# tjhladish/AbcSmc

Hardware: AMD Instinct MI355X
Metric: particles/sec per SMC generation (PLS+weight+resample), 1/2/4/8 GPU (higher is better)
Workload: dtype f64 (inputs, model, distances, proposals, results; pair sums of the weight stage: fp64 operands as three f16 limbs on the matrix pipe + f32 v_exp_f32, weights <= 5e-7 rel of the fp64 oracle, largest seen 3.1e-7); 1 GPU; configs[2]: synthetic 1M particles x 16 params x 32 metrics, PLS 8 components, full generation; particles_per_gpu=1000000, particles_total=1000000, metrics=32, params=16, pls_components=8, pred_prior_size=100000, prev_pred_prior_size=100000, next_set_size=1000000, noise=MULTIVARIATE, ncomp_chosen=8, pls_component_rule=wilcoxon, parallelism=row-sharded x1, launcher=single GPU

## Files before the change

abcsmc_amd/csrc/abc_internal.h:

```cpp
#pragma once
#include <hip/hip_runtime.h>
#include <stddef.h>
#include <stdint.h>
#include <stdio.h>
#include <stdlib.h>
#include <string.h>

#include "../../include/abcsmc_hip.h"

#define ABC_WAVE 64

inline const char* abc_diag_env(const char* name) {
    static const bool on = [] { const char* d = getenv("ABC_DIAG"); return d && d[0] == '1'; }();
    return on ? getenv(name) : nullptr;
}

struct abc_wx_words {
    int left;
    int vmax_lo, vmax_hi;
    int ncomp;
    int changed;
    int decided;
    int n_rest;
    int n_level;
// ... 205 lines not shown
}

int launch_stats_shift(abc_ctx*, const double* X, const double* Y, size_t n, size_t ldx, size_t ldy,
                       size_t M, size_t P, double* stats);
bool abc_gram_takes_i8(const abc_ctx*, const double* X, const double* Y, size_t n, size_t ldx, size_t ldy, size_t M, size_t P,
                       uint64_t n_train_global, size_t n_set);
int launch_stats_accumulate(abc_ctx*, const double* X, const double* Y, size_t n, size_t ldx,
                            size_t ldy, size_t M, size_t P, uint64_t row0, uint64_t n_train_global,
                            double* stats, size_t n_set = 0);
int launch_pls_model(abc_ctx*, const double* stats, const double* obs, size_t M, size_t P, size_t A,
                     int rule, double* model, hipEvent_t done = nullptr);
int launch_simple_model(abc_ctx*, const double* stats, const double* obs, size_t M, size_t P,
                        double* model);
int launch_project_distance(abc_ctx*, const double* X, size_t n, size_t ldx, size_t M, size_t P,
                            size_t A, const double* model, int simple, double* dist);
size_t launch_project_scores(abc_ctx*, const double* X, size_t n, size_t ldx, size_t M, size_t P, size_t A, const double* model, double* S);
int launch_project_distance_scores(abc_ctx*, const double* X, size_t n, size_t ldx, size_t M, size_t P, size_t A, const double* model,
                                   double* dist, double* S, size_t sld, size_t row_test, hipEvent_t done);
int launch_distance_from_scores(abc_ctx*, const double* S, size_t n, size_t sld, size_t M, size_t P, size_t A, const double* model, double* dist);
size_t abc_targets_need(size_t N, size_t A, size_t B, size_t K, bool any_excl);
struct abc_tg_scores { const double* S; size_t sld; const double* O; int KCO; };
int launch_rank_targets(abc_ctx*, const double* X, size_t ldx, const double* Y, size_t ldy, size_t N, size_t M, size_t P,
                        const double* model, size_t A, const double* targets, size_t ldt, size_t B, const uint64_t* exclude,
                        bool any_excl, size_t K, uint64_t* idx, double* dist, double* post_mean, abc_tg_scores* keep = nullptr,
                        const double* om = nullptr);
int launch_row_weights_check(abc_ctx*, const double* w_dev, size_t N, double* out4_dev);
size_t abc_adjust_need(size_t N, size_t A, size_t P, size_t B, size_t K, bool hcorr = false, size_t ridge = 0);
int launch_rank_targets_adjust(abc_ctx*, const double* X, size_t ldx, const double* Y, size_t ldy, size_t N, size_t M, size_t P,
                               const double* model, size_t A, const double* targets, size_t ldt, size_t B, const uint64_t* exclude,
                               bool any_excl, size_t K, int kernel, uint64_t* idx, double* dist, const abc_adjust_out* out,
                               struct abc_adj_keep* keep = nullptr, const struct AbcTf* tf = nullptr,
                               const struct AbcHc* hc = nullptr, const struct AbcRg* rg = nullptr, const double* om = nullptr);
size_t abc_path_need(size_t N, size_t A, size_t P, size_t B, size_t K, size_t T, bool hcorr = false, size_t ridge = 0);
int launch_rank_targets_path(abc_ctx*, const double* X, size_t ldx, const double* Y, size_t ldy, size_t N, size_t M, size_t P,
                             const double* model, size_t A, const double* targets, size_t ldt, size_t B, const uint64_t* exclude,
                             bool any_excl, int kernel, uint64_t* idx, double* dist, const abc_path* path,
                             struct abc_adj_keep* keep = nullptr, const double* Yt = nullptr, const struct AbcTf* tf = nullptr,
                             const struct AbcHc* hc = nullptr, const struct AbcRg* rg = nullptr, const double* om = nullptr);
int launch_param_transf(abc_ctx*, const struct AbcTf* tf, const double* V, size_t ldv, size_t n, size_t P, int inverse, double* out,
                        size_t ldo, unsigned long long* outside);
struct SmValues {
    int method;
    const uint64_t* idx;
    const double* Y;
    size_t ldy;
    const struct abc_adj_keep* adj;
    int A;
    int kernel;
    const double* V;
    size_t ldv;
    const double* w;
    const double* om;
};
size_t abc_summary_need(size_t B, size_t K, size_t P);
int launch_summary(abc_ctx*, const SmValues& sv, size_t B, size_t K, size_t P, const abc_summary* sum);
size_t abc_path_summary_need(size_t B, const size_t* Ks, size_t T, size_t P, int method);
int launch_path_summary(abc_ctx*, const SmValues& sv, size_t B, const size_t* Ks, size_t T, size_t P, const abc_summary* sum);
int abc_summary_check_weights(abc_ctx*, const double* w, size_t K, const char* fn);
size_t abc_density_need(size_t B, size_t K, size_t P, size_t G);
int launch_density(abc_ctx*, const SmValues& sv, size_t B, size_t K, size_t P, const abc_density* dn, const char* fn);
struct DnSeg;
size_t abc_density_segs_need(size_t B, size_t K, size_t P);
int launch_density_segs(abc_ctx*, const SmValues& sv, size_t B, size_t K, size_t P, const abc_density* dn, const DnSeg** segs,
                        const char* fn);
size_t abc_joint_pairs(const abc_joint* jt, size_t P);
size_t abc_joint_need(size_t B, size_t K, size_t P, size_t G, size_t npairs);
int launch_joint(abc_ctx*, const SmValues& sv, size_t B, size_t K, size_t P, const abc_joint* jt, const char* fn);
size_t abc_draws_need(size_t B, size_t K, size_t P, int smooth);
int launch_draws(abc_ctx*, const SmValues& sv, size_t B, size_t K, size_t P, const abc_draws* dr, const char* fn);
int launch_select_smallest(abc_ctx*, const double* dist, size_t n, size_t K, uint64_t idx_base,
                           uint64_t* idx, double* dist_out, bool defer_check = false);
int abc_select_check(abc_ctx* ctx, int* failed);
int abc_select_check_queue(abc_ctx* ctx, int* slot);
int abc_select_check_done(abc_ctx* ctx, const int* slot);
inline size_t abc_kde_slices(size_t kn, size_t Kp, int PP) {
    if (kn == 0 || Kp == 0) return 1;
    size_t rows_per_slice = 24576 / (size_t)PP;
    if (rows_per_slice < 256) rows_per_slice = 256;
    size_t s = (Kp + rows_per_slice - 1) / rows_per_slice;
    const size_t rb = (kn + 255) / 256;
    if (s * rb < 4096) s = (4096 + rb - 1) / rb;
    size_t cap = ((size_t)64 << 20) / (8 * kn);
    if (cap < 8) cap = 8;
    if (s > cap) s = cap;
    if (s > Kp / 64) s = Kp / 64;
    if (s < 1) s = 1;
    if (s > 1024) s = 1024;
    return s;
}
int launch_merge_runs(abc_ctx* ctx, const double* key, const uint64_t* idx, int W, size_t len, double* okey, uint64_t* oidx,
                      uint64_t* osrc = nullptr);
int launch_sort_pairs(abc_ctx*, double* key, uint64_t* idx, size_t n);
int launch_select_begin(abc_ctx*, uint64_t K, long long* state, int* hist);
int launch_select_hist(abc_ctx*, const double* dist, size_t n, const long long* state, int pass, int* hist);
int launch_select_pick(abc_ctx*, long long* state, int pass, int* hist, uint64_t K);
int launch_select_count(abc_ctx*, const double* dist, size_t n, const long long* state, long long* counts);
int launch_select_compact(abc_ctx*, const double* dist, size_t n, const long long* state, uint64_t n_less,
                          uint64_t ties_take, uint64_t idx_base, uint64_t* idx_out, double* dist_out);
int abc_sort_u64_bytes(abc_ctx*, unsigned long long* key0, unsigned long long* val0, unsigned long long* key1,
                       unsigned long long* val1, size_t n, int byte_lo, int byte_hi);
struct abc_wx_shard {
    size_t nv_total;
    const double* nv_ranks;
    size_t nv_stride;
};
bool abc_wx_cascade_applies(size_t nv_total, size_t P, size_t A);
int launch_wilcoxon(abc_ctx*, const double* X, const double* Y, size_t n, size_t ldx, size_t ldy, size_t M, size_t P,
                    size_t A, size_t row_test, double* model, const abc_wx_shard* sh = nullptr, double* dec = nullptr,
                    int* changed_host = nullptr, int stop_at_max = 0);
int launch_wilcoxon_commit(abc_ctx*, double* model, size_t M, size_t P, size_t A, const double* dec, int with_hdr);
struct abc_wx_run;
struct abc_wx_scores_hook { int (*fn)(void* arg, double** S, size_t* sld); void* arg; };
int launch_wilcoxon_begin(abc_ctx*, const double* X, const double* Y, size_t n, size_t ldx, size_t ldy, size_t M, size_t P, size_t A,
                          size_t row_test, double* model, double* dec, int stop_at_max, abc_wx_run** out,
                          const abc_wx_scores_hook* scores = nullptr, int hold_level0 = 0, const abc_wx_shard* sh = nullptr);
int launch_wilcoxon_level0(abc_ctx*, abc_wx_run* run);
int launch_wilcoxon_finish(abc_ctx*, abc_wx_run* run, int* changed_host);
void launch_wilcoxon_abandon(abc_ctx*, abc_wx_run* run, hipStream_t its_stream);
int abc_comm_all_reduce(abc_ctx* ctx, void* buf, size_t count, int dtype);
int abc_comm_all_gather(abc_ctx* ctx, const void* send, void* recv, size_t bytes);
int abc_xbuf_reserve(abc_ctx* ctx, size_t bytes);
int abc_giveups_ensure(abc_ctx* ctx);
int launch_gather_rows(abc_ctx*, const double* Y, size_t n_local, size_t ldy, size_t P,
                       const uint64_t* idx, size_t K, uint64_t idx_base, double* theta, size_t ldt,
                       const int* sel_fail = nullptr, int* sel_fail_pin = nullptr, hipEvent_t done = nullptr);
#define ABC_INTERNAL_RETRY (-2147483647)
int launch_doubled_variance(abc_ctx*, const double* theta, size_t K, size_t P, double* dv);
int launch_theta_stats(abc_ctx*, const double* theta, size_t K, size_t P, double** stats_out);
struct abc_theta_fused {
    double* dv; double* L; int* spd; double* rows ; double* Lpad ;
    const double* model_hdr; double* hdr_pin; int* spd_pin;
};
int launch_post_tail(abc_ctx*, const double* theta, size_t K, size_t P, const double* stats, const abc_theta_fused* f);
int launch_dv_from_stats(abc_ctx*, const double* stats, size_t P, double* dv);
int launch_mvn_from_stats(abc_ctx*, const double* stats, size_t P, double* L, int* status_dev);
struct abc_wprev {
    void* wc ; double* b; double* hb; unsigned short* bt; unsigned* far_list;
    unsigned* tmin;
    size_t Kp, P, kn_max; int split, ready;
};
int launch_weights_prev(abc_ctx*, size_t P, size_t kn_max, const double* theta_prev, size_t Kp, const double* w_prev,
                        const double* dv_prev, abc_wprev* out, hipStream_t st);
int launch_weights_raw(abc_ctx*, const abc_prior* priors, const double* theta, size_t K, size_t P,
                       size_t k0, size_t kn, const double* theta_prev, size_t Kp,
                       const double* w_prev, const double* dv_prev, double* w_raw, const abc_wprev* prev = nullptr,
                       const double** sumsq_out = nullptr);
int abc_weights_prev_early(abc_ctx* ctx, size_t P, size_t kn_max, const double* theta_prev, size_t Kp, const double* w_prev,
                           const double* dv_prev, abc_wprev* out);
int launch_fill(abc_ctx*, double* w, size_t K, double v, hipStream_t st = nullptr);
int launch_normalize_l2(abc_ctx*, double* w, size_t K, double* host_mirror = nullptr, const double* sumsq_parts = nullptr);
static inline size_t abc_alias_pin_bytes(size_t K) { return K * (sizeof(double) * 3 + sizeof(uint32_t) * 3) + 2 * sizeof(uint32_t) + 16; }
int launch_mvn_setup(abc_ctx*, const double* theta, size_t K, size_t P, double* L, int* status_host,
                     int* status_dev);
int launch_resample(abc_ctx*, const abc_rng* rng, const double* w, size_t K, uint64_t i0, size_t n,
                    uint64_t* parent, int (*while_host_builds)(void*) = nullptr, void* hook_arg = nullptr,
                    bool uniform_weights = false, const uint32_t* raw_ready = nullptr, bool weights_on_host = false,
                    const volatile int* abort_flag = nullptr, bool parents_ready = false, int* alias_check_deferred = nullptr);
int abc_rng_streams_early(abc_ctx* ctx, const abc_rng* rng, uint64_t i0, size_t n, uint64_t* seeds, uint64_t seed_stream_offset,
                          uint32_t** raw, uint64_t* parent_uniform = nullptr, size_t K_uniform = 0);
int abc_rng_seeds_early(abc_ctx* ctx, const abc_rng* rng, uint64_t i0, size_t n, uint64_t* seeds, uint64_t seed_stream_offset);
int abc_side_fork(abc_ctx* ctx);
int abc_uniform_alias(abc_ctx* ctx, size_t K);
struct abc_perturb_prep { double* rows; int seeds_done; double* Lpad; };
int launch_perturb_prepare(abc_ctx*, const abc_rng* rng, const double* theta, size_t K, size_t P, uint64_t i0, size_t n,
                           uint64_t* seeds, uint64_t seed_stream_offset, abc_perturb_prep* prep, int multivariate = 0,
                           const double* L_or_dv = nullptr);
static inline int abc_perturb_pp(size_t P) {
    int PP = 2;
    while (PP < (int)P) PP *= 2;
    return (P > 64) ? (int)((P + 63) / 64 * 64) : PP;
}
int launch_perturb(abc_ctx*, const abc_rng* rng, const double* theta, size_t K, size_t P,
                   const abc_prior* priors, const uint64_t* parent, uint64_t i0, size_t n,
                   int multivariate, const double* L_or_dv, double* out, uint64_t* seeds,
                   uint64_t seed_stream_offset, const abc_perturb_prep* prep = nullptr);

struct abc_side_moments { abc_theta_fused out; double* stats; double* L; };
int abc_moments_on_side(abc_ctx* ctx, const double* theta, size_t K, size_t P, bool multivariate, double* L_io, double* dv,
                        int* spd_dev, const double* model_hdr, bool theta_ev_bound, const char* who, abc_side_moments* m);
int abc_normalize_for_resample(abc_ctx* ctx, double* w, size_t K, size_t Nn, const double* sumsq, bool* w_on_host);
struct abc_prep_arg {
    abc_ctx* ctx; const abc_rng* rng; const double* theta; const double* theta_stats; size_t K, P, Nn;
    uint64_t i0, seed_off; uint64_t* seeds; abc_perturb_prep* prep; double* L; int* spd_dev; double* dv; bool moments;
    const double* model_hdr; double* hdr_pin; int* spd_pin;
};
int abc_prep_hook(void* prep_arg);
int abc_alias_repair(abc_ctx* ctx, const abc_rng* rng_entry, const double* w, size_t K, uint64_t i0, size_t Nn, uint64_t seed_off,
                     uint64_t* parent, const double* theta, size_t P, const abc_prior* priors, int multivariate, const double* L_or_dv,
                     double* next, abc_perturb_prep* prep, bool giveups_to_snapshot);

int launch_perturb_reference(abc_ctx*, abc_rng* rng_after_draws, const double* theta, size_t K, size_t P, const abc_prior* priors,
                             const uint64_t* parent, size_t n, int multivariate, const double* L_or_dv, double* out,
                             uint64_t* seeds);

void abc_alias_preproc(size_t K, const double* w, double* F, uint32_t* A, double* E, uint32_t* smalls, uint32_t* bigs, bool knuth = true);

int launch_alias_build_dev(abc_ctx*, const double* w, size_t K, double* F, uint32_t* A, int* fail_dev, int* fail_pin,
                           const int** verdict_src = nullptr);
size_t abc_alias_dev_need(size_t K);
constexpr size_t ABC_ALIAS_DEV_MAX_K = (size_t)2 << 20;
constexpr size_t ABC_ALIAS_DEV_MIN_K = 20000;
constexpr size_t ABC_ALIAS_DEV_SMALL_K = 300000;

size_t abc_ws_need(size_t N, size_t M, size_t P, size_t A, size_t K, size_t Kp, size_t Nnext);
size_t abc_wx_need(size_t n_validation, size_t P, size_t A);
int abc_timing_flush(abc_ctx* ctx);
void abc_comm_release(abc_ctx* ctx);

void taus2_set(abc_rng* r, unsigned long seed);
uint32_t taus2_get(abc_rng* r);
void taus2_jump(abc_rng* r, uint64_t n);
```

abcsmc_amd/csrc/alias_dev.hip:

```cpp
#include <stdlib.h>

#include "abc_internal.h"

namespace {

typedef __int128 i128;
typedef unsigned __int128 u128;
typedef unsigned long long u64;

#ifndef ABC_AL_I
#define ABC_AL_I 4
#endif
#define ABC_AL_CAT2(a, b) a##b
#define ABC_AL_CAT(a, b) ABC_AL_CAT2(a, b)
#define ABC_AL_FN(name) ABC_AL_CAT(name##_i, ABC_AL_I)
constexpr int AL_T = 256;
constexpr int AL_I = ABC_AL_I;
constexpr int AL_B = AL_T * AL_I;
constexpr int AL_MAXBLK = 8192;
constexpr int AL_SUM_BITS = 44;

struct RMap { i128 t0, t1, b; int k; int pad_[3]; };

__device__ __forceinline__ i128 shl(i128 v, int s) { return (i128)((u128)v << s); }
__device__ __forceinline__ int bitlen(i128 v) {
    const u64 hi = (u64)((u128)v >> 64), lo = (u64)v;
    return hi ? 128 - __clzll((long long)hi) : (lo ? 64 - __clzll((long long)lo) : 0);
}
__device__ __forceinline__ int level_of(i128 v) { const int b = bitlen(v); return b > 53 ? b - 53 : 0; }

__device__ __forceinline__ RMap rne_map(int k, i128 c, bool sticky) {
    RMap m;
    m.k = k; m.b = 0; m.pad_[0] = m.pad_[1] = m.pad_[2] = 0;
    if (k == 0) { m.t0 = -c - 1; m.t1 = -c; return m; }
    const i128 P = shl(1, k + 1), h = shl(1, k - 1);
    const i128 t_even = -c - shl(1, k) + h;
    const i128 t_odd = -c + h + (sticky ? 0 : 1);
    m.t0 = t_odd - P; m.t1 = t_even;
    return m;
}
__device__ __forceinline__ RMap rmap_identity() { RMap m; m.k = 0; m.t0 = -1; m.t1 = 0; m.b = 0; m.pad_[0] = m.pad_[1] = m.pad_[2] = 0; return m; }
__device__ __forceinline__ i128 rapply(const RMap& m, i128 y) {
    return shl(((y - m.t0) >> (m.k + 1)) + ((y - m.t1) >> (m.k + 1)), m.k) + m.b;
}
__device__ __forceinline__ i128 inv_min(const RMap& m, i128 v) {
    const i128 a = -((-(v - m.b)) >> m.k);
    if (a & 1) return m.t0 + shl((a + 1) >> 1, m.k + 1);
    return m.t1 + shl(a >> 1, m.k + 1);
}
__device__ __forceinline__ RMap compose(const RMap& m1, const RMap& m2) {
    RMap r;
    if (m2.k < m1.k) { r = m1; r.b = rapply(m2, m1.b); return r; }
    r.k = m2.k; r.t0 = inv_min(m1, m2.t0); r.t1 = inv_min(m1, m2.t1); r.b = m2.b;
    r.pad_[0] = r.pad_[1] = r.pad_[2] = 0;
    return r;
}

__device__ __forceinline__ i128 to_grid(double x, int e0, bool* inexact) {
    const u64 bits = (u64)__double_as_longlong(x);
    const int be = (int)((bits >> 52) & 0x7ff);
    u64 mant = bits & 0xfffffffffffffull;
    int e;
    if (be == 0) { if (mant == 0) return 0; e = -1074; } else { mant |= 1ull << 52; e = be - 1075; }
    const int sh = e - e0;
    if (sh >= 0) return (sh < 70) ? shl((i128)mant, sh) : (i128)0;
    if (sh <= -64) { *inexact = true; return 0; }
    if (mant & ((1ull << -sh) - 1)) *inexact = true;
    return (i128)(mant >> -sh);
}
__device__ __forceinline__ double from_grid(i128 v, int e0, bool* ok) {
    if (v < 0) { *ok = false; return 0.0; }
    if (v == 0) return 0.0;
    const int bl = bitlen(v), sh = bl > 53 ? bl - 53 : 0;
    const u64 top = (u64)(v >> sh);
    if (shl((i128)top, sh) != v) { *ok = false; return 0.0; }
    return ldexp((double)top, sh + e0);
}

__device__ __forceinline__ i128 shfl_up_i128(i128 v, int d) {
    const u64 lo = (u64)__shfl_up((long long)(u64)v, d, 64), hi = (u64)__shfl_up((long long)(u64)((u128)v >> 64), d, 64);
    return (i128)(((u128)hi << 64) | lo);
}
__device__ __forceinline__ RMap shfl_up_map(const RMap& m, int d) {
    RMap r;
    r.t0 = shfl_up_i128(m.t0, d); r.t1 = shfl_up_i128(m.t1, d); r.b = shfl_up_i128(m.b, d); r.k = __shfl_up(m.k, d, 64);
    r.pad_[0] = r.pad_[1] = r.pad_[2] = 0;
    return r;
}
__device__ __forceinline__ RMap block_scan_maps(RMap mine, RMap (*buf)[AL_T], RMap* excl) {
    const int t = threadIdx.x, lane = t & 63, wave = t >> 6;
    RMap inc = mine;
#pragma unroll
    for (int d = 1; d < 64; d <<= 1) {
        const RMap up = shfl_up_map(inc, d);
        if (lane >= d) inc = compose(up, inc);
    }
    RMap exw = shfl_up_map(inc, 1);
    if (lane == 0) exw = rmap_identity();
    if (lane == 63) buf[0][wave] = inc;
    __syncthreads();
    RMap before = rmap_identity();
    for (int w = 0; w < wave; w++) before = compose(before, buf[0][w]);
    __syncthreads();
    *excl = compose(before, exw);
    return compose(before, inc);
}
__device__ __forceinline__ RMap prefix_of_blocks(const RMap* __restrict__ agg, int nb, RMap (*buf)[AL_T]) {
    const int t = threadIdx.x;
    const int per = (nb + AL_T - 1) / AL_T;
    RMap m = rmap_identity();
    for (int j = 0; j < per; j++) { const int b = t * per + j; if (b < nb) m = compose(m, agg[b]); }
    RMap ex;
    (void)block_scan_maps(m, buf, &ex);
    __shared__ RMap s_tot;
    if (t == AL_T - 1) s_tot = compose(ex, m);
    __syncthreads();
    const RMap r = s_tot;
    __syncthreads();
    return r;
}

struct AlHead {
    double approx_total;
    double total;
    int e0_sum;
    int e0;
    unsigned ns, nb;
    unsigned nsteps;
    int fail;
    i128 MEAN;
};

__device__ __forceinline__ void al_fail(AlHead* h) { h->fail = 1; }

__device__ __forceinline__ double block_sum_d(double v, double* sm) {
#pragma unroll
    for (int o = 32; o >= 1; o >>= 1) v += __shfl_xor(v, o, 64);
    __syncthreads();
    if ((threadIdx.x & 63) == 0) sm[threadIdx.x >> 6] = v;
    __syncthreads();
    return (sm[0] + sm[1]) + (sm[2] + sm[3]);
}
__global__ __launch_bounds__(AL_T) void k_al_bsum(const double* __restrict__ w, size_t K, double* __restrict__ bsum, AlHead* __restrict__ head,
                                                  int force_fail) {
    __shared__ double sm[4];
    const size_t base = (size_t)blockIdx.x * AL_B + (size_t)threadIdx.x * AL_I;
    double s = 0.0;
    bool bad = false;
#pragma unroll
    for (int j = 0; j < AL_I; j++) if (base + j < K) { const double x = w[base + j]; s += x; bad = bad || !(x >= 0.0) || !(x < 1.0e300); }
    const double bs = block_sum_d(bad ? (double)NAN : s, sm);
    if (threadIdx.x == 0) bsum[blockIdx.x] = bs;
    if (blockIdx.x == 0 && threadIdx.x == 0) {
        head->approx_total = 0.0; head->total = 0.0; head->e0_sum = 0; head->e0 = 0; head->ns = 0; head->nb = 0; head->nsteps = 0;
        head->fail = force_fail; head->MEAN = 0;
    }
}

__device__ __forceinline__ void approx_prefix(const double* __restrict__ bsum, int nblk, int b, double* sm, double* before, double* all) {
    double pb = 0.0, pa = 0.0;
    for (int j = threadIdx.x; j < nblk; j += AL_T) { const double v = bsum[j]; pa += v; if (j < b) pb += v; }
    *before = block_sum_d(pb, sm);
    *all = block_sum_d(pa, sm);
}

struct SumCtx { double before, all; int e0; };
__device__ __forceinline__ RMap sum_map(double x, double s_approx, int e0, AlHead* head) {
    if (x == 0.0) return rmap_identity();
    int ex;
    (void)frexp(s_approx, &ex);
    int k = ex - e0 - 53;
    if (k < 0) k = 0;
    bool sticky = false;
    const i128 c = to_grid(x, e0, &sticky);
    if (k == 0 && sticky) al_fail(head);
    return rne_map(k, c, sticky);
}
__device__ __forceinline__ double block_excl_prefix_d(double mine, double* sd ) {
    const int t = threadIdx.x;
    sd[t] = mine;
    __syncthreads();
    for (int step = 1; step < AL_T; step <<= 1) {
        const double a = (t >= step) ? sd[t - step] : 0.0;
        __syncthreads();
        sd[t] += a;
        __syncthreads();
    }
    const double ex = t ? sd[t - 1] : 0.0;
    __syncthreads();
    return ex;
}

__global__ __launch_bounds__(AL_T) void k_al_sum_reduce(const double* __restrict__ w, size_t K, const double* __restrict__ bsum, int nblk,
                                                        RMap* __restrict__ agg, RMap* __restrict__ tpre, AlHead* __restrict__ head) {
    __shared__ RMap buf[2][AL_T];
    __shared__ double sd[AL_T];
    __shared__ double sm[4];
    double before, all;
    approx_prefix(bsum, nblk, blockIdx.x, sm, &before, &all);
    int etot;
    (void)frexp(all, &etot);
    const int e0 = etot - 53 - AL_SUM_BITS;
    if (!(all > 0.0) || !(all < 1.0e300)) { if (threadIdx.x == 0) al_fail(head); }
    const size_t base = (size_t)blockIdx.x * AL_B + (size_t)threadIdx.x * AL_I;
    double x[AL_I], ts = 0.0;
#pragma unroll
    for (int j = 0; j < AL_I; j++) { x[j] = (base + j < K) ? w[base + j] : 0.0; ts += x[j]; }
    double run = before + block_excl_prefix_d(ts, sd);
    RMap m = rmap_identity();
#pragma unroll
    for (int j = 0; j < AL_I; j++) { run += x[j]; m = compose(m, sum_map(x[j], run, e0, head)); }
    RMap ex;
    const RMap inc = block_scan_maps(m, buf, &ex);
    tpre[(size_t)blockIdx.x * AL_T + threadIdx.x] = ex;
    if (threadIdx.x == AL_T - 1) agg[blockIdx.x] = inc;
    if (blockIdx.x == 0 && threadIdx.x == 0) { head->approx_total = all; head->e0_sum = e0; }
}

__global__ __launch_bounds__(AL_T) void k_al_sum_apply(const double* __restrict__ w, size_t K, const double* __restrict__ bsum, int nblk,
                                                       const RMap* __restrict__ agg, const RMap* __restrict__ tpre, AlHead* __restrict__ head) {
    __shared__ RMap buf[2][AL_T];
    __shared__ double sd[AL_T];
    __shared__ double sm[4];
    double before, all;
    approx_prefix(bsum, nblk, blockIdx.x, sm, &before, &all);
    int etot;
    (void)frexp(all, &etot);
    const int e0 = etot - 53 - AL_SUM_BITS;
    const RMap pre = prefix_of_blocks(agg, blockIdx.x, buf);
    const size_t base = (size_t)blockIdx.x * AL_B + (size_t)threadIdx.x * AL_I;
    double x[AL_I], ts = 0.0;
#pragma unroll
    for (int j = 0; j < AL_I; j++) { x[j] = (base + j < K) ? w[base + j] : 0.0; ts += x[j]; }
    double run = before + block_excl_prefix_d(ts, sd);
    RMap mj[AL_I];
#pragma unroll
    for (int j = 0; j < AL_I; j++) { run += x[j]; mj[j] = sum_map(x[j], run, e0, head); }
    const RMap ex = tpre[(size_t)blockIdx.x * AL_T + threadIdx.x];
    i128 v = rapply(ex, rapply(pre, 0));
    bool ok = true;
    double prev = from_grid(v, e0, &ok);
#pragma unroll
    for (int j = 0; j < AL_I; j++) {
        if (base + j < K) {
            v = rapply(mj[j], v);
            const double c = from_grid(v, e0, &ok);
            if (prev + x[j] != c) ok = false;
            prev = c;
            if (base + j == K - 1) head->total = c;
        }
    }
    if (!ok) al_fail(head);
}

__global__ __launch_bounds__(AL_T) void k_al_classify(const double* __restrict__ w, size_t K, double mean, AlHead* __restrict__ head,
                                                      double* __restrict__ E, unsigned* __restrict__ cnt, double* __restrict__ F,
                                                      uint32_t* __restrict__ A) {
    __shared__ unsigned sc[4];
    const double total = head->total;
    const size_t base = (size_t)blockIdx.x * AL_B + (size_t)threadIdx.x * AL_I;
    unsigned c = 0;
#pragma unroll
    for (int j = 0; j < AL_I; j++) {
        const size_t k = base + j;
        if (k < K) {
            const double e = w[k] / total;
            E[k] = e;
            c += (e < mean) ? 1u : 0u;
            F[k] = 1.0;
            A[k] = (uint32_t)k;
        }
    }
#pragma unroll
    for (int o = 32; o >= 1; o >>= 1) c += __shfl_xor(c, o, 64);
    if ((threadIdx.x & 63) == 0) sc[threadIdx.x >> 6] = c;
    __syncthreads();
    if (threadIdx.x == 0) cnt[blockIdx.x] = sc[0] + sc[1] + sc[2] + sc[3];
    if (blockIdx.x == 0 && threadIdx.x == 0) {
        int em;
        (void)frexp(mean, &em);
        const int e0 = em - 53 - 1;
        bool inexact = false;
        head->e0 = e0;
        head->MEAN = to_grid(mean, e0, &inexact);
        if (!(total > 0.0) || !(total < 1.0e300)) al_fail(head);
    }
}

__global__ __launch_bounds__(AL_T) void k_al_lists(const double* __restrict__ E, size_t K, double mean, const unsigned* __restrict__ cnt,
                                                   int nblk, AlHead* __restrict__ head, uint32_t* __restrict__ sidx, u64* __restrict__ dI,
                                                   uint32_t* __restrict__ bidx, i128* __restrict__ VI) {
    __shared__ unsigned su[AL_T];
    __shared__ unsigned s_before, s_all;
    const int t = threadIdx.x;
    unsigned pb = 0, pa = 0;
    for (int j = t; j < nblk; j += AL_T) { const unsigned v = cnt[j]; pa += v; if (j < (int)blockIdx.x) pb += v; }
    su[t] = pb; __syncthreads();
    for (int s = AL_T / 2; s > 0; s >>= 1) { if (t < s) su[t] += su[t + s]; __syncthreads(); }
    if (t == 0) s_before = su[0];
    __syncthreads();
    su[t] = pa; __syncthreads();
    for (int s = AL_T / 2; s > 0; s >>= 1) { if (t < s) su[t] += su[t + s]; __syncthreads(); }
    if (t == 0) s_all = su[0];
    __syncthreads();
    const unsigned ns = s_all, nb = (unsigned)K - ns;
    const int e0 = head->e0;
    const size_t base = (size_t)blockIdx.x * AL_B + (size_t)t * AL_I;
    unsigned mine = 0;
    double e[AL_I];
#pragma unroll
    for (int j = 0; j < AL_I; j++) { e[j] = (base + j < K) ? E[base + j] : 0.0; if (base + j < K && e[j] < mean) mine++; }
    su[t] = mine; __syncthreads();
    for (int step = 1; step < AL_T; step <<= 1) {
        const unsigned a = (t >= step) ? su[t - step] : 0u;
        __syncthreads();
        su[t] += a;
        __syncthreads();
    }
    unsigned rs = s_before + su[t] - mine;
    bool bad = false;
#pragma unroll
    for (int j = 0; j < AL_I; j++) {
        const size_t k = base + j;
        if (k >= K) break;
        if (e[j] < mean) {
            const unsigned pos = ns - 1 - rs;
            bool inexact = false;
            const double d = mean - e[j];
            sidx[pos] = (uint32_t)k;
            dI[pos] = (u64)to_grid(d, e0, &inexact);
            bad = bad || inexact || !(e[j] >= 0.0);
            rs++;
        } else {
            const unsigned rb = (unsigned)k - rs;
            const unsigned pos = nb - 1 - rb;
            bool inexact = false;
            bidx[pos] = (uint32_t)k;
            VI[pos] = to_grid(e[j], e0, &inexact);
            bad = bad || inexact || !(e[j] <= 2.0);
        }
    }
    if (bad) al_fail(head);
    if (blockIdx.x == 0 && t == 0) { head->ns = ns; head->nb = nb; head->nsteps = 0; }
}

__device__ __forceinline__ i128 block_sum_i(i128 v, i128* sh ) {
    const int t = threadIdx.x;
    sh[t] = v; __syncthreads();
    for (int s = AL_T / 2; s > 0; s >>= 1) { if (t < s) sh[t] += sh[t + s]; __syncthreads(); }
    const i128 r = sh[0];
    __syncthreads();
    return r;
}
__global__ __launch_bounds__(AL_T) void k_al_psum_reduce(const u64* __restrict__ dI, const i128* __restrict__ VI, const AlHead* __restrict__ head,
                                                         i128* __restrict__ bs , int nblk) {
    __shared__ i128 sh[AL_T];
    const bool bigs = blockIdx.y == 1;
    const size_t n = bigs ? head->nb : head->ns;
    const i128 MEAN = head->MEAN;
    const size_t base = (size_t)blockIdx.x * AL_B + (size_t)threadIdx.x * AL_I;
    i128 s = 0;
#pragma unroll
    for (int j = 0; j < AL_I; j++) if (base + j < n) s += bigs ? (VI[base + j] - MEAN) : (i128)dI[base + j];
    const i128 tot = block_sum_i(s, sh);
    if (threadIdx.x == 0) bs[(size_t)blockIdx.y * nblk + blockIdx.x] = tot;
}
__global__ __launch_bounds__(AL_T) void k_al_psum_apply(const u64* __restrict__ dI, const i128* __restrict__ VI, const AlHead* __restrict__ head,
                                                        const i128* __restrict__ bs, int nblk, i128* __restrict__ D, i128* __restrict__ X,
                                                        i128* __restrict__ Dc, i128* __restrict__ Xc ) {
    __shared__ i128 sh[AL_T];
    const bool bigs = blockIdx.y == 1;
    const size_t n = bigs ? head->nb : head->ns;
    if ((size_t)blockIdx.x * AL_B >= n) return;
    const i128 MEAN = head->MEAN;
    const int t = threadIdx.x;
    i128 pb = 0;
    for (int j = t; j < (int)blockIdx.x; j += AL_T) pb += bs[(size_t)blockIdx.y * nblk + j];
    const i128 before = block_sum_i(pb, sh);
    const size_t base = (size_t)blockIdx.x * AL_B + (size_t)t * AL_I;
    i128 v[AL_I], ts = 0;
#pragma unroll
    for (int j = 0; j < AL_I; j++) { v[j] = (base + j < n) ? (bigs ? (VI[base + j] - MEAN) : (i128)dI[base + j]) : (i128)0; ts += v[j]; }
    sh[t] = ts; __syncthreads();
    for (int step = 1; step < AL_T; step <<= 1) {
        const i128 a = (t >= step) ? sh[t - step] : (i128)0;
        __syncthreads();
        sh[t] += a;
        __syncthreads();
    }
    i128 run = before + sh[t] - ts;
    i128* out = bigs ? X : D;
#pragma unroll
    for (int j = 0; j < AL_I; j++) if (base + j < n) { run += v[j]; out[base + j] = run; }
    if (t == AL_T - 1) (bigs ? Xc : Dc)[blockIdx.x] = run;
}

constexpr unsigned AL_HAND = 0x80000000u;
struct StepRec { i128 val; uint32_t idx; unsigned char k1, k2; unsigned char pad_[10]; };
template <bool STRICT>
__device__ __forceinline__ unsigned rank_two_level(const i128* __restrict__ a, const i128* __restrict__ c, unsigned n, i128 v) {
    const unsigned nblk = (n + AL_B - 1) / AL_B;
    unsigned lo = 0, hi = nblk;
    while (lo < hi) { const unsigned mid = (lo + hi) >> 1; const i128 x = c[mid]; if (STRICT ? (x < v) : (x <= v)) lo = mid + 1; else hi = mid; }
    if (lo >= nblk) return n;
    unsigned l2 = lo * AL_B, h2 = l2 + AL_B;
    if (h2 > n) h2 = n;
    while (l2 < h2) { const unsigned mid = (l2 + h2) >> 1; const i128 x = a[mid]; if (STRICT ? (x < v) : (x <= v)) l2 = mid + 1; else h2 = mid; }
    return l2;
}

__global__ __launch_bounds__(AL_T) void k_al_structure(const i128* __restrict__ D, const i128* __restrict__ X, const i128* __restrict__ Dc,
                                                       const i128* __restrict__ Xc, const u64* __restrict__ dI, const i128* __restrict__ VI,
                                                       AlHead* __restrict__ head, uint32_t* __restrict__ z, uint32_t* __restrict__ jof,
                                                       StepRec* __restrict__ step) {
    if (head->fail) return;
    const unsigned ns = head->ns, nb = head->nb;
    const size_t t = (size_t)blockIdx.x * AL_T + threadIdx.x;
    unsigned pos = 0;
    if (ns != 0 && nb != 0 && t < (size_t)ns + nb) {
        if (t < ns) {
            const unsigned i = (unsigned)t + 1;
            const i128 dprev = (i >= 2) ? D[i - 2] : (i128)0;
            const unsigned j = rank_two_level<true>(X, Xc, nb, dprev) + 1;
            jof[i - 1] = j;
            if (j <= nb) {
                pos = i + j - 1;
                const i128 star = head->MEAN + X[j - 1] - D[i - 1];
                StepRec r;
                r.val = (i128)dI[i - 1]; r.idx = i - 1; r.k1 = (unsigned char)level_of(star < 0 ? (i128)0 : star); r.k2 = 0;
                step[pos - 1] = r;
            }
        } else {
            const unsigned j = (unsigned)(t - ns) + 1;
            const i128 xj = X[j - 1];
            const unsigned zz = rank_two_level<false>(D, Dc, ns, xj) + 1;
            z[j - 1] = zz;
            if (zz <= ns && j < nb) {
                pos = zz + j;
                const i128 dz = D[zz - 1];
                const i128 dd = dz - xj;
                const i128 star = head->MEAN + X[j] - dz;
                StepRec r;
                r.val = VI[j]; r.idx = AL_HAND | (j - 1);
                r.k1 = (unsigned char)level_of(dd < 0 ? (i128)0 : dd); r.k2 = (unsigned char)level_of(star < 0 ? (i128)0 : star);
                step[pos - 1] = r;
            }
        }
    }
    __shared__ unsigned smax[4];
#pragma unroll
    for (int o = 32; o >= 1; o >>= 1) { const unsigned v = __shfl_xor(pos, o, 64); pos = v > pos ? v : pos; }
    if ((threadIdx.x & 63) == 0) smax[threadIdx.x >> 6] = pos;
    __syncthreads();
    if (threadIdx.x == 0) {
        unsigned m = smax[0];
        for (int w = 1; w < 4; w++) m = smax[w] > m ? smax[w] : m;
        if (m) atomicMax(&head->nsteps, m);
    }
}

struct ServeArgs {
    const double* E; const uint32_t* sidx; const uint32_t* bidx; const u64* dI; const i128* VI; const i128* D; const i128* X;
    const uint32_t* z; const uint32_t* jof; const StepRec* step;
};
__device__ __forceinline__ RMap serve_map(const StepRec& r, i128 MEAN) {
    if (!(r.idx & AL_HAND)) return rne_map(r.k1, -r.val, false);
    const RMap m1 = rne_map(r.k1, -MEAN, false);
    const RMap m2 = rne_map(r.k2, r.val, false);
    return compose(m1, m2);
}

__global__ __launch_bounds__(AL_T) void k_al_serve_reduce(ServeArgs a, const AlHead* __restrict__ head, RMap* __restrict__ agg,
                                                          RMap* __restrict__ tpre) {
    __shared__ RMap buf[2][AL_T];
    const unsigned n = head->nsteps;
    if (head->fail) return;
    if ((size_t)blockIdx.x * AL_B >= n) { if (threadIdx.x == 0) agg[blockIdx.x] = rmap_identity(); return; }
    const size_t base = (size_t)blockIdx.x * AL_B + (size_t)threadIdx.x * AL_I;
    const i128 MEAN = head->MEAN;
    StepRec rec[AL_I];
#pragma unroll
    for (int j = 0; j < AL_I; j++) if (base + j < n) rec[j] = a.step[base + j];
    RMap m = rmap_identity();
#pragma unroll
    for (int j = 0; j < AL_I; j++) if (base + j < n) m = compose(m, serve_map(rec[j], MEAN));
    RMap ex;
    const RMap inc = block_scan_maps(m, buf, &ex);
    tpre[(size_t)blockIdx.x * AL_T + threadIdx.x] = ex;
    if (threadIdx.x == AL_T - 1) agg[blockIdx.x] = inc;
}

__global__ __launch_bounds__(AL_T) void k_al_serve_apply(ServeArgs a, AlHead* __restrict__ head, const RMap* __restrict__ agg,
                                                         const RMap* __restrict__ tpre, double mean,
                                                         double dK, double* __restrict__ F, uint32_t* __restrict__ A, int* __restrict__ fail_out,
                                                         int* __restrict__ fail_pin) {
    __shared__ RMap buf[2][AL_T];
    const unsigned n = head->nsteps, ns = head->ns, nb = head->nb;
    const bool last_block = ((size_t)(blockIdx.x + 1) * AL_B >= n);
    if ((size_t)blockIdx.x * AL_B >= n && blockIdx.x != 0) return;
    if (n == 0 || head->fail) {
        if (blockIdx.x == 0 && threadIdx.x == 0) { *fail_out = head->fail; if (fail_pin) *fail_pin = head->fail; }
        return;
    }
    const RMap pre = prefix_of_blocks(agg, blockIdx.x, buf);
    const size_t base = (size_t)blockIdx.x * AL_B + (size_t)threadIdx.x * AL_I;
    const i128 MEAN = head->MEAN;
    StepRec rec[AL_I];
    RMap mj[AL_I];
#pragma unroll
    for (int j = 0; j < AL_I; j++) {
        if (base + j < n) { rec[j] = a.step[base + j]; mj[j] = serve_map(rec[j], MEAN); }
        else { rec[j].idx = 0; mj[j] = rmap_identity(); }
    }
    const RMap ex = tpre[(size_t)blockIdx.x * AL_T + threadIdx.x];
    const int e0 = head->e0;
    i128 v = rapply(ex, rapply(pre, a.VI[0]));
    bool ok = true;
    double prev = from_grid(v, e0, &ok);
#pragma unroll
    for (int j = 0; j < AL_I; j++) {
        const size_t t = base + j;
        if (t >= n) break;
        v = rapply(mj[j], v);
        const double c = from_grid(v, e0, &ok);
        const uint32_t s = rec[j].idx;
        unsigned jcur;
        bool below, at_last_small;
        if (!(s & AL_HAND)) {
            const unsigned ii = s;
            jcur = a.jof[ii];
            const uint32_t sm = a.sidx[ii];
            const double es = a.E[sm];
            if (prev - (mean - es) != c) ok = false;
            below = (a.z[jcur - 1] == ii + 1);
            at_last_small = (ii + 1 == ns);
            A[sm] = a.bidx[jcur - 1];
            F[sm] = dK * es;
        } else {
            const unsigned j0 = (s & ~AL_HAND) + 1;
            jcur = j0 + 1;
            const uint32_t bo = a.bidx[j0 - 1], bn = a.bidx[j0];
            const double dd = mean - prev;
            if (a.E[bn] - dd != c) ok = false;
            const unsigned zz = a.z[j0 - 1];
            below = (a.z[j0] == zz);
            at_last_small = (zz == ns);
            A[bo] = bn;
            F[bo] = dK * prev;
        }
        if (!(jcur == nb && at_last_small)) {
            if (below) { if (!(c < mean)) ok = false; }
            else if (!(c > mean)) ok = false;
        }
        prev = c;
    }
    if (!ok) al_fail(head);
    (void)last_block;
}
__global__ void k_al_flag(const AlHead* __restrict__ head, int* __restrict__ fail_out, int* __restrict__ fail_pin) {
    if (threadIdx.x == 0) { *fail_out = head->fail; if (fail_pin) *fail_pin = head->fail; }
}

}

#if ABC_AL_I == 4
int launch_alias_build_dev_i2(abc_ctx* ctx, const double* w, size_t K, double* F, uint32_t* A, int* fail_dev, int* fail_pin,
                              const int** verdict_src);
int launch_alias_build_dev_i4(abc_ctx* ctx, const double* w, size_t K, double* F, uint32_t* A, int* fail_dev, int* fail_pin,
                              const int** verdict_src);
size_t abc_alias_dev_need(size_t K) {
    constexpr size_t B = AL_T * 2;
    const size_t nblk = (K + B - 1) / B + 1, nblk2 = (2 * K + B - 1) / B + 1;
    return K * (8 + 4 + 4 + 8 + 16 + 16 + 16 + 4 + 4 + 64) + nblk * (8 + 4 + 64 + 64) + nblk2 * 64 * (AL_T + 1) + sizeof(AlHead) + 64 * 256;
}
int launch_alias_build_dev(abc_ctx* ctx, const double* w, size_t K, double* F, uint32_t* A, int* fail_dev, int* fail_pin,
                           const int** verdict_src) {
    if (K <= ABC_ALIAS_DEV_SMALL_K) return launch_alias_build_dev_i2(ctx, w, K, F, A, fail_dev, fail_pin, verdict_src);
    return launch_alias_build_dev_i4(ctx, w, K, F, A, fail_dev, fail_pin, verdict_src);
}
#endif

int ABC_AL_FN(launch_alias_build_dev)(abc_ctx* ctx, const double* w, size_t K, double* F, uint32_t* A, int* fail_dev, int* fail_pin,
                                      const int** verdict_src) {
    if (K == 0 || K > (size_t)AL_MAXBLK * AL_B / 2) ABC_FAIL(ctx, ABC_ERR_UNSUPPORTED, "device alias build: K = %zu", K);
    const int nblk = (int)((K + AL_B - 1) / AL_B), nblk2 = (int)((2 * K + AL_B - 1) / AL_B);
    AlHead* head = (AlHead*)abc_ws_alloc(ctx, sizeof(AlHead));
    double* bsum = (double*)abc_ws_alloc(ctx, (size_t)nblk * 8);
    RMap* agg = (RMap*)abc_ws_alloc(ctx, (size_t)(nblk2 > nblk ? nblk2 : nblk) * sizeof(RMap));
    RMap* tpre = (RMap*)abc_ws_alloc(ctx, (size_t)(nblk2 > nblk ? nblk2 : nblk) * AL_T * sizeof(RMap));
    double* E = (double*)abc_ws_alloc(ctx, K * 8);
    unsigned* cnt = (unsigned*)abc_ws_alloc(ctx, (size_t)nblk * 4);
    uint32_t* sidx = (uint32_t*)abc_ws_alloc(ctx, K * 4);
    uint32_t* bidx = (uint32_t*)abc_ws_alloc(ctx, K * 4);
    u64* dI = (u64*)abc_ws_alloc(ctx, K * 8);
    i128* VI = (i128*)abc_ws_alloc(ctx, K * 16);
    i128* D = (i128*)abc_ws_alloc(ctx, K * 16);
    i128* X = (i128*)abc_ws_alloc(ctx, K * 16);
    i128* bs = (i128*)abc_ws_alloc(ctx, (size_t)4 * nblk * 16);
    i128* Dc = bs ? bs + (size_t)2 * nblk : nullptr;
    i128* Xc = bs ? bs + (size_t)3 * nblk : nullptr;
    uint32_t* z = (uint32_t*)abc_ws_alloc(ctx, K * 4);
    uint32_t* jof = (uint32_t*)abc_ws_alloc(ctx, K * 4);
    StepRec* step = (StepRec*)abc_ws_alloc(ctx, 2 * K * sizeof(StepRec));
    if (!head || !bsum || !agg || !tpre || !E || !cnt || !sidx || !bidx || !dI || !VI || !D || !X || !bs || !z || !jof || !step)
        ABC_FAIL(ctx, ABC_ERR_NOMEM, "device alias build: workspace exhausted");
    const double mean = 1.0 / (double)K, dK = (double)K;
    hipStream_t st = ctx->stream;
    const int force_fail = abc_diag_env("ABC_ALIAS_FORCE_FAIL") ? 1 : 0;
    hipLaunchKernelGGL(k_al_bsum, dim3(nblk), dim3(AL_T), 0, st, w, K, bsum, head, force_fail);
    hipLaunchKernelGGL(k_al_sum_reduce, dim3(nblk), dim3(AL_T), 0, st, w, K, (const double*)bsum, nblk, agg, tpre, head);
    hipLaunchKernelGGL(k_al_sum_apply, dim3(nblk), dim3(AL_T), 0, st, w, K, (const double*)bsum, nblk, (const RMap*)agg, (const RMap*)tpre, head);
    hipLaunchKernelGGL(k_al_classify, dim3(nblk), dim3(AL_T), 0, st, w, K, mean, head, E, cnt, F, A);
    hipLaunchKernelGGL(k_al_lists, dim3(nblk), dim3(AL_T), 0, st, (const double*)E, K, mean, (const unsigned*)cnt, nblk, head, sidx, dI, bidx, VI);
    hipLaunchKernelGGL(k_al_psum_reduce, dim3(nblk, 2), dim3(AL_T), 0, st, (const u64*)dI, (const i128*)VI, (const AlHead*)head, bs, nblk);
    hipLaunchKernelGGL(k_al_psum_apply, dim3(nblk, 2), dim3(AL_T), 0, st, (const u64*)dI, (const i128*)VI, (const AlHead*)head,
                       (const i128*)bs, nblk, D, X, Dc, Xc);
    hipLaunchKernelGGL(k_al_structure, dim3((unsigned)((K + AL_T - 1) / AL_T)), dim3(AL_T), 0, st, (const i128*)D, (const i128*)X, (const i128*)Dc, (const i128*)Xc, (const u64*)dI, (const i128*)VI, head, z, jof, step);
    ServeArgs a = {E, sidx, bidx, dI, VI, D, X, z, jof, step};
    hipLaunchKernelGGL(k_al_serve_reduce, dim3(nblk2), dim3(AL_T), 0, st, a, (const AlHead*)head, agg, tpre);
    hipLaunchKernelGGL(k_al_serve_apply, dim3(nblk2), dim3(AL_T), 0, st, a, head, (const RMap*)agg, (const RMap*)tpre, mean, dK, F, A, fail_dev, fail_pin);
    if (verdict_src) *verdict_src = &head->fail;
    else hipLaunchKernelGGL(k_al_flag, dim3(1), dim3(64), 0, st, (const AlHead*)head, fail_dev, fail_pin);
    ABC_HIP(ctx, hipGetLastError());
    return ABC_OK;
}
```

abcsmc_amd/csrc/api.hip:

```cpp
#include <math.h>
#include <stdlib.h>

#include <new>
#include <vector>

#include "abc_internal.h"
#include "adjust_dev.h"

int abc_ws_reserve(abc_ctx* ctx, size_t bytes) {
    bytes = abc_align(bytes, 1 << 20);
    if (bytes > ctx->ws_bytes) {
        ABC_HIP(ctx, hipStreamSynchronize(ctx->stream));
        if (ctx->ws) { ABC_HIP(ctx, hipFree(ctx->ws)); ctx->ws = nullptr; ctx->ws_bytes = 0; }
        ABC_HIP(ctx, hipMalloc((void**)&ctx->ws, bytes));
        ctx->ws_bytes = bytes;
    }
    ctx->ws_off = 0;
    static const char* poison = abc_diag_env("ABC_WS_POISON");
    if (poison && ctx->ws) ABC_HIP(ctx, hipMemsetAsync(ctx->ws, (int)strtol(poison, nullptr, 16), ctx->ws_bytes, ctx->stream));
    return ABC_OK;
}
void* abc_ws_alloc(abc_ctx* ctx, size_t bytes) {
    const size_t off = abc_align(ctx->ws_off, 256);
    if (off + bytes > ctx->ws_bytes) return nullptr;
// ... 919 lines not shown
            &sarg};
        {
            StreamScope on_wx(ctx, ctx->wx_stream);
            ABC_TRY(launch_wilcoxon_begin(ctx, io->X, io->Y, N, N, N, M, P, A, (size_t)ntrain, model, wx_dec, 1, &wx_run, &hook,
                                          1));
        }
        projected = sarg.dist == nullptr;
        scores_all = projected ? sarg.S_all : nullptr;
    } else if (wx_rule)
        ABC_TRY(launch_wilcoxon(ctx, io->X, io->Y, N, N, N, M, P, A, (size_t)ntrain, model));
    if (!projected) ABC_TRY(launch_project_distance(ctx, io->X, N, N, M, simple ? Pstat : P, A, model, simple, dist));
    if (K == 0) return ABC_OK;
    ABC_TRY(launch_select_smallest(ctx, dist, N, K, 0, io->idx, io->dist, io->w != nullptr));
    if (!simple && ncomp_host && !io->w) {
        double hdr[4];
        ABC_HIP(ctx, hipMemcpyAsync(hdr, model, sizeof(hdr), hipMemcpyDeviceToHost, ctx->stream));
        ABC_HIP(ctx, hipStreamSynchronize(ctx->stream));
        *ncomp_host = (int32_t)hdr[0];
    }
    if (!io->w) return ABC_OK;

    double* theta = io->theta ? io->theta : (double*)abc_ws_alloc(ctx, K * P * 8);
    if (!theta) ABC_FAIL(ctx, ABC_ERR_NOMEM, "generation: workspace exhausted");
    int* pfail_early = &ctx->status_pin->gather_sel_fail;
    *pfail_early = 0;
    volatile unsigned* pgaveup = &ctx->status_pin->giveup_flag;
    *pgaveup = 0u;
    double* const hdr_pin = ctx->status_pin->model_hdr;
    int* const spd_pin = &ctx->status_pin->spd;
    hdr_pin[0] = 0.0; *spd_pin = 0;
    bool status_early = false;
    bool bins_deferred = ctx->sel_bins_ran && ctx->sel_fail_dev && !ctx->sel_force_radix;
    ctx->side_early_waited = false;
    if (wprev.ready) {
        ABC_HIP(ctx, hipStreamWaitEvent(ctx->stream, ctx->ev_prev, 0));
        ctx->side_early_waited = true;
    }
    const bool defer_moments = Nn && P <= 64 && K >= 2;
    const bool moments_side_planned = defer_moments && !uniform_w && ctx->side && ctx->noise_mode != ABC_NOISE_REFERENCE_STREAM;
    if (moments_side_planned && !ctx->ev_theta) {
        ABC_HIP(ctx, hipEventCreateWithFlags(&ctx->ev_theta, abc_xstream_event_flags()));
        ABC_HIP(ctx, hipEventCreateWithFlags(&ctx->ev_moments, abc_xstream_event_flags()));
    }
    const bool theta_ev_bound = moments_side_planned;
    ABC_TRY(launch_gather_rows(ctx, io->Y, N, N, P, io->idx, K, 0, theta, K, bins_deferred ? ctx->sel_fail_dev : nullptr, pfail_early,
                               theta_ev_bound ? ctx->ev_theta : nullptr));
    if (wx_run) {
        StreamScope on_wx(ctx, ctx->wx_stream);
        ABC_TRY(launch_wilcoxon_level0(ctx, wx_run));
    }
    bool wx_tail_pending = false;
    if (wx_spec) {
        int changed = 2, rc;
        {
            StreamScope on_wx(ctx, ctx->wx_stream);
            rc = launch_wilcoxon_finish(ctx, wx_run, &changed);
            wx_run = nullptr;
            if (rc == ABC_OK && hipEventRecord(ctx->ev_wx_done, ctx->wx_stream) != hipSuccess) rc = ABC_ERR_HIP;
        }
        if (rc == ABC_INTERNAL_RETRY) {
            ABC_HIP(ctx, hipStreamSynchronize(ctx->wx_stream));
            ABC_HIP(ctx, hipStreamSynchronize(ctx->stream));
            rc = launch_wilcoxon(ctx, io->X, io->Y, N, N, N, M, P, A, (size_t)ntrain, model);
            changed = 2;
        }
        if (rc != ABC_OK) { if (!ctx->err[0]) snprintf(ctx->err, sizeof(ctx->err), "generation: the component rule's reduction failed"); return rc; }
        if (changed == 1) {
            ABC_HIP(ctx, hipStreamWaitEvent(ctx->stream, ctx->ev_wx_done, 0));
            ABC_TRY(launch_wilcoxon_commit(ctx, model, M, P, A, wx_dec, 1));
        } else if (changed == 0) {
            StreamScope on_wx(ctx, ctx->wx_stream);
            ABC_TRY(launch_wilcoxon_commit(ctx, model, M, P, A, wx_dec, 0));
            wx_tail_pending = true;
        }
        if (changed) {
            ctx->wx_moved_counts++;
            pfail_early = &ctx->status_pin->repeat_sel_fail;
            *pfail_early = 0;
            if (scores_all) ABC_TRY(launch_distance_from_scores(ctx, scores_all, N, N, M, P, A, model, dist));
            else ABC_TRY(launch_project_distance(ctx, io->X, N, N, M, P, A, model, 0, dist));
            ABC_TRY(launch_select_smallest(ctx, dist, N, K, 0, io->idx, io->dist, true));
            bins_deferred = ctx->sel_bins_ran && ctx->sel_fail_dev && !ctx->sel_force_radix;
            ABC_TRY(launch_gather_rows(ctx, io->Y, N, N, P, io->idx, K, 0, theta, K, bins_deferred ? ctx->sel_fail_dev : nullptr, pfail_early,
                                       theta_ev_bound ? ctx->ev_theta : nullptr));
        }
    }
    auto repeat_with_radix = [&]() -> int {
        ABC_HIP(ctx, hipStreamSynchronize(ctx->stream));
        if (ctx->side) ABC_HIP(ctx, hipStreamSynchronize(ctx->side));
        if (ctx->wx_stream) ABC_HIP(ctx, hipStreamSynchronize(ctx->wx_stream));
        if (ctx->giveups_dev)
            ABC_HIP(ctx, hipMemcpyAsync(ctx->giveups_dev, ctx->giveups_dev + 1, sizeof(unsigned long long), hipMemcpyDeviceToDevice, ctx->stream));
        ctx->sel_bins_ran = false;
        ctx->ws_off = ws_entry;
        if (rng) *rng = rng_entry;
        ctx->generation_repeats++;
        const bool radix0 = ctx->sel_force_radix;
        ctx->sel_force_radix = true;
        const int rc = generation_core(ctx, cfg, io, rng, ncomp_host, simple, model_out);
        ctx->sel_force_radix = radix0;
        return rc;
    };
    double* dv = io->dv ? io->dv : (double*)abc_ws_alloc(ctx, P * 8);
    double* theta_stats = nullptr;
    if (defer_moments) {
    } else if (P <= 64 && K >= 2) {
        StageTimer tm(ctx, ST_GATHER_DV);
        ABC_TRY(launch_theta_stats(ctx, theta, K, P, &theta_stats));
        ABC_TRY(launch_dv_from_stats(ctx, theta_stats, P, dv));
    } else {
        ABC_TRY(launch_doubled_variance(ctx, theta, K, P, dv));
    }
    bool w_on_host = false;
    if (Kp == 0 || !io->theta_prev) {
        if (!filled_early) ABC_TRY(launch_fill(ctx, io->w, K, 1.0 / (double)K));
    } else {
        if (wprev.ready && !ctx->side_early_waited) ABC_HIP(ctx, hipStreamWaitEvent(ctx->stream, ctx->ev_prev, 0));
        const double* sumsq = nullptr;
        ABC_TRY(launch_weights_raw(ctx, io->priors, theta, K, P, 0, K, io->theta_prev, Kp, io->w_prev, io->dv_prev,
                                   io->w, &wprev, &sumsq));
        ABC_TRY(abc_normalize_for_resample(ctx, io->w, K, Nn, sumsq, &w_on_host));
    }
    abc_side_moments side = {};
    bool moments_on_side = false, seeds_waited = false;
    if (moments_side_planned) {
        ABC_TRY(abc_moments_on_side(ctx, theta, K, P, cfg->multivariate != 0, io->L, dv, spd_dev, simple ? nullptr : model, theta_ev_bound,
                                    "generation", &side));
        theta_stats = side.stats;
        moments_on_side = status_early = true;
    }
    int spd = 0;
    bool have_spd = false;
    int alias_deferred = 0;
    uint64_t* parent_used = nullptr;
    double* L_used = nullptr;
    abc_perturb_prep prep_used = {nullptr, 0, nullptr};
    if (Nn) {
        uint64_t* parent = parent_early ? parent_early : (io->parent ? io->parent : (uint64_t*)abc_ws_alloc(ctx, Nn * 8));
        if (!parent) ABC_FAIL(ctx, ABC_ERR_NOMEM, "generation: workspace exhausted");
        double* L = nullptr;
        if (cfg->multivariate) {
            L = side.L ? side.L : (io->L ? io->L : (double*)abc_ws_alloc(ctx, P * P * 8));
            have_spd = true;
        }
        abc_perturb_prep prep = {side.out.rows, (early && io->seeds) ? 1 : 0, side.out.Lpad};
        if (moments_on_side) { ABC_HIP(ctx, hipStreamWaitEvent(ctx->stream, ctx->ev_moments, 0)); seeds_waited = true; }
        const bool hook_moments = defer_moments && !moments_on_side;
        abc_prep_arg pa = {ctx, rng, theta, theta_stats, K, P, Nn, 0, Nn, io->seeds, &prep, moments_on_side ? nullptr : L, spd_dev, dv,
                           hook_moments, nullptr, nullptr, nullptr};
        if (hook_moments) {
            pa.model_hdr = simple ? nullptr : model; pa.hdr_pin = hdr_pin; pa.spd_pin = L ? spd_pin : nullptr;
            status_early = true;
        }
        {
            const int rc = launch_resample(ctx, rng, io->w, K, 0, Nn, parent, abc_prep_hook, &pa, uniform_w, raw_early, w_on_host,
                                           bins_deferred ? pfail_early : nullptr, parent_early != nullptr,
                                           ctx->noise_mode == ABC_NOISE_REFERENCE_STREAM ? nullptr : &alias_deferred);
            if (rc == ABC_INTERNAL_RETRY) return repeat_with_radix();
            ABC_TRY(rc);
        }
        if (ctx->noise_mode == ABC_NOISE_REFERENCE_STREAM) {
            taus2_jump(rng, (uint64_t)Nn);
            ABC_TRY(launch_perturb_reference(ctx, rng, theta, K, P, io->priors, parent, Nn, cfg->multivariate,
                                             cfg->multivariate ? L : dv, io->next, io->seeds));
        } else {
            ABC_TRY(launch_perturb(ctx, rng, theta, K, P, io->priors, parent, 0, Nn, cfg->multivariate,
                                   cfg->multivariate ? L : dv, io->next, io->seeds, Nn, &prep));
            parent_used = parent; L_used = L; prep_used = prep;
            taus2_jump(rng, 2 * (uint64_t)Nn);
        }
    }
    {
        double* hdr = ctx->status_pin->model_hdr;
        int* pspd = &ctx->status_pin->spd;
        int* pfail = &ctx->status_pin->sel_fail;
        if (!status_early) { hdr[0] = 0.0; *pspd = 0; }
        *pfail = 0;
        if (seeds_late && !seeds_waited) ABC_HIP(ctx, hipStreamWaitEvent(ctx->stream, ctx->ev_side, 0));
        const int* fail_dev = (ctx->sel_bins_ran && ctx->sel_fail_dev) ? (const int*)ctx->sel_fail_dev : nullptr;
        unsigned long long* pgive = &ctx->status_pin->giveups;
        *pgive = 0;
        if (!status_early) {
            hipLaunchKernelGGL(k_status_words, dim3(1), dim3(64), 0, ctx->stream, simple ? (const double*)nullptr : (const double*)model,
                               have_spd ? (const int*)spd_dev : (const int*)nullptr, fail_dev, (const unsigned long long*)ctx->giveups_dev, hdr, pspd,
                               pfail, pgive);
            ABC_HIP(ctx, hipGetLastError());
        }
        ctx->side_early_waited = false;
        ABC_HIP(ctx, hipStreamSynchronize(ctx->stream));
        if (wx_tail_pending) ABC_HIP(ctx, hipStreamSynchronize(ctx->wx_stream));
        if (status_early) {
            *pfail = fail_dev ? *(volatile int*)pfail_early : 0;
        } else {
            ctx->giveups_dev_known = *(volatile unsigned long long*)pgive;
        }
        if (ncomp_host) *ncomp_host = (int32_t)hdr[0];
        spd = *pspd;
        const int failed = abc_select_check_done(ctx, pfail);
        if (failed && !ctx->sel_force_radix) return repeat_with_radix();
        if (alias_deferred && *(volatile int*)&ctx->status_pin->alias_fail && parent_used) {
            ABC_TRY(abc_alias_repair(ctx, &rng_entry, io->w, K, 0, Nn, Nn, parent_used, theta, P, io->priors, cfg->multivariate,
                                     cfg->multivariate ? L_used : dv, io->next, &prep_used, true));
        }
    }
    if (ctx->timing && ctx->nev > 128) ABC_TRY(abc_timing_flush(ctx));
    if (spd) ABC_FAIL(ctx, ABC_ERR_NOT_SPD, "covariance of the selected particles is not positive definite");
    {
        if (status_early) {
            if (*pgaveup && ctx->giveups_dev) {
                unsigned long long now = 0;
                ABC_HIP(ctx, hipMemcpyAsync(&now, ctx->giveups_dev, sizeof(now), hipMemcpyDeviceToHost, ctx->stream));
                ABC_HIP(ctx, hipStreamSynchronize(ctx->stream));
                ctx->giveups_dev_known = now;
            }
            *(volatile unsigned long long*)&ctx->status_pin->giveups = ctx->giveups_dev_known;
        }
        const unsigned long long gv = *(volatile unsigned long long*)&ctx->status_pin->giveups + ctx->giveups_host;
        const unsigned long long before = ctx->giveups_seen;
        ctx->giveups_seen = gv;
        ctx->giveups_last_call = (Nn && gv > before) ? gv - before : 0ull;
    }
    return ABC_OK;
}

extern "C" int abc_generation_dev(abc_ctx* ctx, const abc_generation_cfg* cfg, const abc_generation_io* io, abc_rng* rng,
                                  int32_t* ncomp_host) {
    CHECK_CTX(ctx);
    if (!cfg || !io || !io->X || !io->obs || !io->idx) ABC_FAIL(ctx, ABC_ERR_INVALID, "generation: null argument");
    const size_t A = default_A(cfg->M, cfg->P, cfg->max_comp);
    size_t need = abc_ws_need(cfg->N, cfg->M, cfg->P, A, cfg->K, cfg->Kp, cfg->Nnext);
    if (cfg->rule == ABC_RULE_WILCOXON) need += abc_wx_need(cfg->N, cfg->P, A) + cfg->N * A * 8 + 4096;
    ABC_TRY(abc_ws_reserve(ctx, need));
    return generation_core(ctx, cfg, io, rng, ncomp_host, 0);
}

namespace {
struct Stage {
    abc_ctx* ctx;
    bool full = false;
    template <typename T>
    T* up(const T* h, size_t n) {
        T* d = dev<T>(n);
        if (d && h && n) (void)hipMemcpyAsync(d, h, n * sizeof(T), hipMemcpyHostToDevice, ctx->stream);
        return d;
    }
    template <typename T>
    T* dev(size_t n) {
        T* d = (T*)abc_ws_alloc(ctx, n * sizeof(T));
        if (!d) full = true;
        return d;
    }
    template <typename T>
    void down(T* h, const T* d, size_t n) {
        if (h && d && n) (void)hipMemcpyAsync(h, d, n * sizeof(T), hipMemcpyDeviceToHost, ctx->stream);
    }
};
}

static int ranking_host(abc_ctx* ctx, const double* X, const double* Y, const double* obs, size_t N, size_t M,
                        size_t P, double train_frac, int max_comp, int rule, size_t K, uint64_t* idx, double* dist,
                        int32_t* ncomp, double* R, double* mean, double* sd, int simple) {
    if (!X || !obs || !idx || (!simple && !Y)) ABC_FAIL(ctx, ABC_ERR_INVALID, "ranking: null argument");
    const size_t A = simple ? 0 : default_A(M, P, max_comp);
    ABC_TRY(abc_ws_reserve(ctx, abc_ws_need(N, M, P, A, K, 0, 0) + (N * (M + P) + M + 2 * K) * 8 +
                                    ((!simple && rule == ABC_RULE_WILCOXON) ? abc_wx_need(N, P, A) : 0)));
    Stage s{ctx};
    abc_generation_io io;
    memset(&io, 0, sizeof(io));
    io.X = s.up(X, N * M);
    io.Y = simple ? nullptr : s.up(Y, N * P);
    io.obs = s.up(obs, M);
    io.idx = s.dev<uint64_t>(K);
    io.dist = s.dev<double>(K);
    if (!io.X || !io.obs || !io.idx || !io.dist) ABC_FAIL(ctx, ABC_ERR_NOMEM, "ranking: workspace exhausted");
    abc_generation_cfg cfg;
    memset(&cfg, 0, sizeof(cfg));
    cfg.N = N; cfg.M = M; cfg.P = simple ? 0 : P; cfg.K = K; cfg.train_frac = train_frac;
    cfg.max_comp = max_comp; cfg.rule = rule;
    const double* model = nullptr;
    ABC_TRY(generation_core(ctx, &cfg, &io, nullptr, ncomp, simple, &model));
    s.down(idx, io.idx, K);
    s.down(dist, io.dist, K);
    if (R || mean || sd) {
        const ModelLayout ML = model_layout(M, simple ? 0 : P, A);
        if (R && !simple) s.down(R, model + ML.off_R, M * A);
        s.down(mean, model + ML.off_mean, M);
        s.down(sd, model + ML.off_sd, M);
    }
    ABC_HIP(ctx, hipStreamSynchronize(ctx->stream));
    ABC_HIP(ctx, hipGetLastError());
    return ABC_OK;
}

extern "C" int abc_particle_ranking_pls(abc_ctx* ctx, const double* X, const double* Y, const double* obs, size_t N,
                                        size_t M, size_t P, double train_frac, int max_comp, int rule, size_t K,
                                        uint64_t* idx, double* dist, int32_t* ncomp, double* R, double* mean,
                                        double* sd) {
    CHECK_CTX(ctx);
    return ranking_host(ctx, X, Y, obs, N, M, P, train_frac, max_comp, rule, K, idx, dist, ncomp, R, mean, sd, 0);
}

extern "C" int abc_particle_ranking_simple(abc_ctx* ctx, const double* X, const double* obs, size_t N, size_t M,
                                           size_t K, uint64_t* idx, double* dist) {
    CHECK_CTX(ctx);
    return ranking_host(ctx, X, nullptr, obs, N, M, 0, 1.0, 0, 0, K, idx, dist, nullptr, nullptr, nullptr, nullptr, 1);
}

extern "C" int abc_calculate_doubled_variance(abc_ctx* ctx, const double* theta, size_t K, size_t P, double* dv) {
    CHECK_CTX(ctx);
    if (!theta || !dv) ABC_FAIL(ctx, ABC_ERR_INVALID, "doubled_variance: null argument");
    ABC_TRY(abc_ws_reserve(ctx, (K * P + P) * 8 + (1 << 20)));
    Stage s{ctx};
    double* dth = s.up(theta, K * P);
    double* ddv = s.dev<double>(P);
    ABC_TRY(launch_doubled_variance(ctx, dth, K, P, ddv));
    s.down(dv, ddv, P);
    ABC_HIP(ctx, hipStreamSynchronize(ctx->stream));
    return ABC_OK;
}

extern "C" int abc_weight_predictive_prior_uniform(abc_ctx* ctx, size_t K, double* w) {
    CHECK_CTX(ctx);
    if (!w || !K) ABC_FAIL(ctx, ABC_ERR_INVALID, "weights: null argument");
    ABC_TRY(abc_ws_reserve(ctx, K * 8 + (1 << 20)));
    Stage s{ctx};
    double* dw = s.dev<double>(K);
    ABC_TRY(launch_fill(ctx, dw, K, 1.0 / (double)K));
    s.down(w, dw, K);
    ABC_HIP(ctx, hipStreamSynchronize(ctx->stream));
    return ABC_OK;
}

extern "C" int abc_weight_predictive_prior(abc_ctx* ctx, const abc_prior* priors, const double* theta, size_t K,
                                           size_t P, const double* theta_prev, size_t Kp, const double* w_prev,
                                           const double* dv_prev, double* w) {
    CHECK_CTX(ctx);
    if (!priors || !theta || !theta_prev || !w_prev || !dv_prev || !w)
        ABC_FAIL(ctx, ABC_ERR_INVALID, "weights: null argument");
    ABC_TRY(abc_ws_reserve(ctx, abc_ws_need(0, 1, P, 1, K, Kp, 0) + ((K + Kp) * (P + 1) + 2 * P) * 8 + P * sizeof(abc_prior)));
    Stage s{ctx};
    abc_prior* dpr = s.up(priors, P);
    double* dth = s.up(theta, K * P);
    double* dtp = s.up(theta_prev, Kp * P);
    double* dwp = s.up(w_prev, Kp);
    double* ddv = s.up(dv_prev, P);
    double* dw = s.dev<double>(K);
    if (!dpr || !dth || !dtp || !dwp || !ddv || !dw) ABC_FAIL(ctx, ABC_ERR_NOMEM, "weights: workspace exhausted");
    ABC_TRY(launch_weights_raw(ctx, dpr, dth, K, P, 0, K, dtp, Kp, dwp, ddv, dw));
    ABC_TRY(launch_normalize_l2(ctx, dw, K));
    s.down(w, dw, K);
    ABC_HIP(ctx, hipStreamSynchronize(ctx->stream));
    return ABC_OK;
}

extern "C" int abc_setup_mvn_sampler(abc_ctx* ctx, const double* theta, size_t K, size_t P, double* L) {
    CHECK_CTX(ctx);
    if (!theta || !L) ABC_FAIL(ctx, ABC_ERR_INVALID, "mvn: null argument");
    ABC_TRY(abc_ws_reserve(ctx, abc_ws_need(0, P, 0, 1, 0, 0, 0) + (K * P + P * P) * 8));
    Stage s{ctx};
    double* dth = s.up(theta, K * P);
    double* dL = s.dev<double>(P * P);
    int st = 0;
    ABC_TRY(launch_mvn_setup(ctx, dth, K, P, dL, &st, nullptr));
    if (st) ABC_FAIL(ctx, ABC_ERR_NOT_SPD, "covariance of the selected particles is not positive definite");
    s.down(L, dL, P * P);
    ABC_HIP(ctx, hipStreamSynchronize(ctx->stream));
    return ABC_OK;
}

extern "C" int abc_sample_posterior(abc_ctx* ctx, abc_rng* rng, const double* w, size_t K, size_t n, uint64_t* idx) {
    CHECK_CTX(ctx);
    if (!rng || !w || !idx) ABC_FAIL(ctx, ABC_ERR_INVALID, "sample_posterior: null argument");
    ABC_TRY(abc_ws_reserve(ctx, abc_ws_need(0, 1, 1, 1, 0, 0, n) + K * 8 + n * 8 + abc_alias_dev_need(K)));
    Stage s{ctx};
    double* dw = s.up(w, K);
    uint64_t* dp = s.dev<uint64_t>(n);
    ABC_TRY(launch_resample(ctx, rng, dw, K, 0, n, dp));
    s.down(idx, dp, n);
    ABC_HIP(ctx, hipStreamSynchronize(ctx->stream));
    taus2_jump(rng, n);
    return ABC_OK;
}

extern "C" int abc_alias_table(abc_ctx* ctx, const double* w, size_t K, double* F, uint64_t* A, int* on_device) {
    CHECK_CTX(ctx);
    if (!w || !F || !A || !K || K > 0xffffffffull) ABC_FAIL(ctx, ABC_ERR_INVALID, "alias table: null argument or K = %zu", K);
    if (on_device) *on_device = 0;
    std::vector<double> hF(K);
    std::vector<uint32_t> hA(K);
    bool done = false;
    if (ctx->alias_mode == ABC_ALIAS_DEVICE && K >= 2 && K <= ABC_ALIAS_DEV_MAX_K) {
        ABC_TRY(abc_ws_reserve(ctx, abc_alias_dev_need(K) + K * 20 + (1u << 20)));
        Stage s{ctx};
        double* dw = s.up(w, K);
        double* dF = s.dev<double>(K);
        uint32_t* dA = s.dev<uint32_t>(K);
        int* dfail = s.dev<int>(1);
        if (!dw || !dF || !dA || !dfail) ABC_FAIL(ctx, ABC_ERR_NOMEM, "alias table: workspace exhausted");
        ABC_TRY(launch_alias_build_dev(ctx, dw, K, dF, dA, dfail, nullptr));
        int fail = 0;
        ctx->alias_dev_builds++;
        s.down(hF.data(), (const double*)dF, K);
        s.down(hA.data(), (const uint32_t*)dA, K);
        s.down(&fail, (const int*)dfail, 1);
        ABC_HIP(ctx, hipStreamSynchronize(ctx->stream));
        if (fail) ctx->alias_dev_fallbacks++; else done = true;
        if (done && on_device) *on_device = 1;
    }
    if (!done) {
        std::vector<double> E(K);
        std::vector<uint32_t> S(K + 1), B(K + 1);
        abc_alias_preproc(K, w, hF.data(), hA.data(), E.data(), S.data(), B.data(), false);
    }
    const double dK = (double)K;
    for (size_t k = 0; k < K; k++) { F[k] = (hF[k] + (double)k) / dK; A[k] = hA[k]; }
    return ABC_OK;
}

static int sample_host(abc_ctx* ctx, abc_rng* rng, size_t n, const double* w, const double* theta, size_t K, size_t P,
                       const abc_prior* priors, const double* L_or_dv, int multivariate, double* out, uint64_t* parent,
                       uint64_t* seeds) {
    if (!rng || !w || !theta || !priors || !L_or_dv || !out) ABC_FAIL(ctx, ABC_ERR_INVALID, "sample: null argument");
    ABC_TRY(abc_ws_reserve(ctx, abc_ws_need(0, 1, P, 1, K, 0, n) + (K * (P + 1) + P * P + n * (P + 2)) * 8 + P * sizeof(abc_prior)));
    Stage s{ctx};
    double* dw = s.up(w, K);
    double* dth = s.up(theta, K * P);
    abc_prior* dpr = s.up(priors, P);
    double* dl = s.up(L_or_dv, multivariate ? P * P : P);
    double* dout = s.dev<double>(n * P);
    uint64_t* dpar = s.dev<uint64_t>(n);
    uint64_t* dseed = seeds ? s.dev<uint64_t>(n) : nullptr;
    if (!dw || !dth || !dpr || !dl || !dout || !dpar) ABC_FAIL(ctx, ABC_ERR_NOMEM, "sample: workspace exhausted");
    ABC_TRY(launch_resample(ctx, rng, dw, K, 0, n, dpar));
    if (ctx->noise_mode == ABC_NOISE_REFERENCE_STREAM) {
        taus2_jump(rng, (uint64_t)n);
        ABC_TRY(launch_perturb_reference(ctx, rng, dth, K, P, dpr, dpar, n, multivariate, dl, dout, dseed));
    } else {
        ABC_TRY(launch_perturb(ctx, rng, dth, K, P, dpr, dpar, 0, n, multivariate, dl, dout, dseed, n));
        taus2_jump(rng, seeds ? 2 * (uint64_t)n : (uint64_t)n);
    }
    s.down(out, dout, n * P);
    s.down(parent, dpar, n);
    s.down(seeds, dseed, n);
    ABC_HIP(ctx, hipStreamSynchronize(ctx->stream));
    return ABC_OK;
}

extern "C" int abc_sample_mvn_predictive_priors(abc_ctx* ctx, abc_rng* rng, size_t n, const double* w,
                                                const double* theta, size_t K, size_t P, const abc_prior* priors,
                                                const double* L, double* out, uint64_t* parent, uint64_t* seeds) {
    CHECK_CTX(ctx);
    return sample_host(ctx, rng, n, w, theta, K, P, priors, L, 1, out, parent, seeds);
}

extern "C" int abc_sample_predictive_priors(abc_ctx* ctx, abc_rng* rng, size_t n, const double* w, const double* theta,
                                            size_t K, size_t P, const abc_prior* priors, const double* dv, double* out,
                                            uint64_t* parent, uint64_t* seeds) {
    CHECK_CTX(ctx);
    return sample_host(ctx, rng, n, w, theta, K, P, priors, dv, 0, out, parent, seeds);
}

static int summary_check(abc_ctx* ctx, const char* fn, const abc_summary* sum) {
    if (!sum) ABC_FAIL(ctx, ABC_ERR_INVALID, "%s: null argument (sum is required)", fn);
    if (sum->nq == 0 || sum->nq > 64) ABC_FAIL(ctx, ABC_ERR_INVALID, "%s: nq = %zu levels (1 to 64)", fn, sum->nq);
    if (!sum->probs) ABC_FAIL(ctx, ABC_ERR_INVALID, "%s: null argument (probs is required)", fn);
    for (size_t q = 0; q < sum->nq; q++)
        if (!(sum->probs[q] >= 0.0 && sum->probs[q] <= 1.0))
            ABC_FAIL(ctx, ABC_ERR_INVALID, "%s: probs[%zu] = %g is not a level in [0, 1]", fn, q, sum->probs[q]);
    if (sum->cdf && !sum->truth) ABC_FAIL(ctx, ABC_ERR_INVALID, "%s: cdf requires truth", fn);
    return ABC_OK;
}

static int density_check(abc_ctx* ctx, const char* fn, const abc_density* den) {
    if (!den) ABC_FAIL(ctx, ABC_ERR_INVALID, "%s: null argument (den is required)", fn);
    if (den->G < 2 || den->G > 4096) ABC_FAIL(ctx, ABC_ERR_INVALID, "%s: G = %zu grid points (2 to 4096)", fn, den->G);
    if (!(den->cut >= 0.0) || !std::isfinite(den->cut)) ABC_FAIL(ctx, ABC_ERR_INVALID, "%s: cut = %g (finite, >= 0)", fn, den->cut);
    if (!(den->bw_scale > 0.0) || !std::isfinite(den->bw_scale))
        ABC_FAIL(ctx, ABC_ERR_INVALID, "%s: bw_scale = %g (finite, > 0)", fn, den->bw_scale);
    if (!den->dens && !den->grid && !den->bw_out && !den->mode && !den->mode_dens)
        ABC_FAIL(ctx, ABC_ERR_INVALID, "%s: every output member of den is NULL", fn);
    return ABC_OK;
}

static int joint_check(abc_ctx* ctx, const char* fn, const abc_joint* jt, size_t P) {
    if (!jt) ABC_FAIL(ctx, ABC_ERR_INVALID, "%s: null argument (jt is required)", fn);
    if (jt->G < 2 || jt->G > 256) ABC_FAIL(ctx, ABC_ERR_INVALID, "%s: G = %zu grid points per axis (2 to 256)", fn, jt->G);
    if (!(jt->cut >= 0.0) || !std::isfinite(jt->cut)) ABC_FAIL(ctx, ABC_ERR_INVALID, "%s: cut = %g (finite, >= 0)", fn, jt->cut);
    if (!(jt->bw_scale > 0.0) || !std::isfinite(jt->bw_scale))
        ABC_FAIL(ctx, ABC_ERR_INVALID, "%s: bw_scale = %g (finite, > 0)", fn, jt->bw_scale);
    if (jt->pairs) {
        if (jt->npairs == 0) ABC_FAIL(ctx, ABC_ERR_INVALID, "%s: pairs given with npairs == 0", fn);
        if (jt->npairs > ((size_t)1 << 22)) ABC_FAIL(ctx, ABC_ERR_UNSUPPORTED, "%s: npairs = %zu (at most 2^22)", fn, jt->npairs);
        for (size_t p = 0; p < jt->npairs; p++) {
            const int32_t i = jt->pairs[2 * p], j = jt->pairs[2 * p + 1];
            if (i < 0 || j < 0 || (size_t)i >= P || (size_t)j >= P || i == j)
                ABC_FAIL(ctx, ABC_ERR_INVALID, "%s: pairs[%zu] = (%d, %d) is not a pair of two of the %zu parameters", fn, p, (int)i,
                         (int)j, P);
        }
    }
    if (!jt->mean && !jt->cov && !jt->corr && !jt->dens && !jt->grid && !jt->bw_out && !jt->mode && !jt->mode_dens)
        ABC_FAIL(ctx, ABC_ERR_INVALID, "%s: every output member of jt is NULL", fn);
    return ABC_OK;
}

static int draws_check(abc_ctx* ctx, const char* fn, const abc_draws* dr) {
    if (!dr) ABC_FAIL(ctx, ABC_ERR_INVALID, "%s: null argument (dr is required)", fn);
    if (dr->S == 0 || dr->S > ((size_t)1 << 24)) ABC_FAIL(ctx, ABC_ERR_INVALID, "%s: S = %zu draws per target (1 to 2^24)", fn, dr->S);
    if (dr->smooth != 0 && dr->smooth != 1)
        ABC_FAIL(ctx, ABC_ERR_INVALID, "%s: smooth %d (0 = weighted, 1 = smoothed bootstrap)", fn, dr->smooth);
    if (dr->smooth && (!(dr->bw_scale > 0.0) || !std::isfinite(dr->bw_scale)))
        ABC_FAIL(ctx, ABC_ERR_INVALID, "%s: bw_scale = %g (finite, > 0)", fn, dr->bw_scale);
    if (!dr->draws && !dr->src && !dr->bw_out && !dr->ess) ABC_FAIL(ctx, ABC_ERR_INVALID, "%s: every output member of dr is NULL", fn);
    return ABC_OK;
}

static abc_summary summary_stage(Stage& s, const abc_summary* h, size_t G, size_t P) {
    abc_summary d = *h;
    d.truth = h->truth ? s.up(h->truth, G * P) : nullptr;
    d.quant = h->quant ? s.dev<double>(G * h->nq * P) : nullptr;
    d.cdf = h->cdf ? s.dev<double>(G * P) : nullptr;
    return d;
}
static void summary_down(Stage& s, const abc_summary* h, const abc_summary& d, size_t G, size_t P) {
    s.down(h->quant, d.quant, G * h->nq * P);
    s.down(h->cdf, d.cdf, G * P);
}

static abc_density density_stage(Stage& s, const abc_density* h, size_t ns) {
    abc_density d = *h;
    d.bw = h->bw ? s.up(h->bw, ns) : nullptr;
    d.dens = h->dens ? s.dev<double>(ns * h->G) : nullptr;
    d.grid = h->grid ? s.dev<double>(ns * 2) : nullptr;
    d.bw_out = h->bw_out ? s.dev<double>(ns) : nullptr;
    d.mode = h->mode ? s.dev<double>(ns) : nullptr;
    d.mode_dens = h->mode_dens ? s.dev<double>(ns) : nullptr;
    return d;
}
static void density_down(Stage& s, const abc_density* h, const abc_density& d, size_t ns) {
    s.down(h->dens, d.dens, ns * h->G);
    s.down(h->grid, d.grid, ns * 2);
    s.down(h->bw_out, d.bw_out, ns);
    s.down(h->mode, d.mode, ns);
    s.down(h->mode_dens, d.mode_dens, ns);
}

static size_t joint_stage_bytes(const abc_joint* h, size_t B, size_t P) {
    const size_t np = abc_joint_pairs(h, P);
    return B * (P * (2 * P + 5) + np * ((h->dens ? h->G * h->G : 0) + 3)) * 8 + 40 * 256;
}
static abc_joint joint_stage(Stage& s, const abc_joint* h, size_t B, size_t P) {
    const size_t np = abc_joint_pairs(h, P);
    abc_joint d = *h;
    d.bw = h->bw ? s.up(h->bw, B * P) : nullptr;
    d.mean = h->mean ? s.dev<double>(B * P) : nullptr;
    d.cov = h->cov ? s.dev<double>(B * P * P) : nullptr;
    d.corr = h->corr ? s.dev<double>(B * P * P) : nullptr;
    d.dens = (h->dens && np) ? s.dev<double>(B * np * h->G * h->G) : nullptr;
    d.grid = h->grid ? s.dev<double>(B * P * 2) : nullptr;
    d.bw_out = h->bw_out ? s.dev<double>(B * P) : nullptr;
    d.mode = (h->mode && np) ? s.dev<double>(B * np * 2) : nullptr;
    d.mode_dens = (h->mode_dens && np) ? s.dev<double>(B * np) : nullptr;
    return d;
}
static void joint_down(Stage& s, const abc_joint* h, const abc_joint& d, size_t B, size_t P) {
    const size_t np = abc_joint_pairs(h, P);
    s.down(h->mean, d.mean, B * P);
    s.down(h->cov, d.cov, B * P * P);
    s.down(h->corr, d.corr, B * P * P);
    s.down(h->dens, d.dens, B * np * h->G * h->G);
    s.down(h->grid, d.grid, B * P * 2);
    s.down(h->bw_out, d.bw_out, B * P);
    s.down(h->mode, d.mode, B * np * 2);
    s.down(h->mode_dens, d.mode_dens, B * np);
}

static abc_draws draws_stage(Stage& s, const abc_draws* h, size_t B, size_t P) {
    abc_draws d = *h;
    d.bw = (h->smooth && h->bw) ? s.up(h->bw, B * P) : nullptr;
    d.draws = h->draws ? s.dev<double>(B * h->S * P) : nullptr;
    d.src = h->src ? s.dev<uint64_t>(B * h->S) : nullptr;
    d.bw_out = h->bw_out ? s.dev<double>(B * P) : nullptr;
    d.ess = h->ess ? s.dev<double>(B) : nullptr;
    return d;
}
static void draws_down(Stage& s, const abc_draws* h, const abc_draws& d, size_t B, size_t P) {
    s.down(h->draws, d.draws, B * h->S * P);
    s.down(h->src, d.src, B * h->S);
    s.down(h->bw_out, d.bw_out, B * P);
    s.down(h->ess, d.ess, B);
}

// ... 643 lines not shown
```

abcsmc_amd/csrc/resample.hip:

```cpp
#include <chrono>
#include <vector>

#include "abc_internal.h"
#include "philox_dev.h"
#include "refstream_host.h"

static inline uint32_t taus_c1(uint32_t s) { return ((s & 4294967294u) << 12) ^ (((s << 13) ^ s) >> 19); }
static inline uint32_t taus_c2(uint32_t s) { return ((s & 4294967288u) << 4) ^ (((s << 2) ^ s) >> 25); }
static inline uint32_t taus_c3(uint32_t s) { return ((s & 4294967280u) << 17) ^ (((s << 3) ^ s) >> 11); }

uint32_t taus2_get(abc_rng* r) {
    r->s1 = taus_c1(r->s1); r->s2 = taus_c2(r->s2); r->s3 = taus_c3(r->s3);
    return r->s1 ^ r->s2 ^ r->s3;
}
void taus2_set(abc_rng* r, unsigned long seed) {
    uint32_t s = (uint32_t)(seed & 0xffffffffUL);
    if (s == 0) s = 1;
    r->s1 = 69069u * s;     if (r->s1 < 2) r->s1 += 2;
    r->s2 = 69069u * r->s1; if (r->s2 < 8) r->s2 += 8;
    r->s3 = 69069u * r->s2; if (r->s3 < 16) r->s3 += 16;
    for (int i = 0; i < 6; i++) taus2_get(r);
}

struct BitMat { uint32_t col[32]; };
static inline uint32_t bm_apply(const BitMat& m, uint32_t v) {
    uint32_t y = 0;
    for (int i = 0; i < 32; i++) y ^= (uint32_t)(-(int32_t)((v >> i) & 1u)) & m.col[i];
    return y;
}
static inline BitMat bm_mul(const BitMat& a, const BitMat& b) {
    BitMat c;
    for (int i = 0; i < 32; i++) c.col[i] = bm_apply(a, b.col[i]);
    return c;
}
static void taus_step_mats(BitMat m[3]) {
    for (int i = 0; i < 32; i++) {
        m[0].col[i] = taus_c1(1u << i); m[1].col[i] = taus_c2(1u << i); m[2].col[i] = taus_c3(1u << i);
    }
}
struct TausPow2 {
    BitMat tab[64][3];
    TausPow2() {
        taus_step_mats(tab[0]);
        for (int k = 1; k < 64; k++)
            for (int c = 0; c < 3; c++) tab[k][c] = bm_mul(tab[k - 1][c], tab[k - 1][c]);
    }
};
static const BitMat (*taus_pow2())[3] {
    static const TausPow2 t;
    return t.tab;
}
void taus2_jump(abc_rng* r, uint64_t n) {
    const BitMat(*tab)[3] = taus_pow2();
    for (int k = 0; k < 64; k++)
        if ((n >> k) & 1ull) {
            r->s1 = bm_apply(tab[k][0], r->s1); r->s2 = bm_apply(tab[k][1], r->s2); r->s3 = bm_apply(tab[k][2], r->s3);
        }
}

namespace {

constexpr int RUN = 64;
constexpr int RUN_LOG2 = 6;

__device__ __forceinline__ uint32_t d_apply(const uint32_t* __restrict__ col, uint32_t v) {
    uint32_t y = 0;
#pragma unroll
    for (int i = 0; i < 32; i++) y ^= (uint32_t)(-(int32_t)((v >> i) & 1u)) & col[i];
    return y;
}

__global__ __launch_bounds__(256) void k_taus_stream(abc_rng base, size_t n, const uint32_t* __restrict__ jt,
                                                     uint32_t* __restrict__ out) {
    __shared__ uint32_t sjt[24 * 96];
    for (int e = threadIdx.x; e < 24 * 96; e += blockDim.x) sjt[e] = jt[e];
    __syncthreads();
    const size_t t = (size_t)blockIdx.x * blockDim.x + threadIdx.x;
    const size_t first = t * RUN;
    if (first >= n) return;
    uint32_t s1 = base.s1, s2 = base.s2, s3 = base.s3;
    for (int k = 0; k < 32; k++)
        if ((t >> k) & 1) {
            const uint32_t* m = (k < 24) ? sjt + k * 96 : jt + (size_t)k * 96;
            s1 = d_apply(m, s1); s2 = d_apply(m + 32, s2); s3 = d_apply(m + 64, s3);
        }
    const size_t last = (first + RUN < n) ? first + RUN : n;
    for (size_t i = first; i < last; i++) {
        s1 = ((s1 & 4294967294u) << 12) ^ (((s1 << 13) ^ s1) >> 19);
        s2 = ((s2 & 4294967288u) << 4) ^ (((s2 << 2) ^ s2) >> 25);
        s3 = ((s3 & 4294967280u) << 17) ^ (((s3 << 3) ^ s3) >> 11);
        out[i] = s1 ^ s2 ^ s3;
    }
}

__global__ __launch_bounds__(256) void k_alias_draw(const uint32_t* __restrict__ raw, size_t n,
                                                    const double* __restrict__ F, const uint32_t* __restrict__ A,
                                                    size_t K, unsigned long long* __restrict__ parent,
                                                    const int* __restrict__ verdict_src = nullptr, int* __restrict__ verdict_dev = nullptr,
                                                    int* __restrict__ verdict_pin = nullptr) {
    const size_t i = (size_t)blockIdx.x * 256 + threadIdx.x;
    if (i == 0 && verdict_src) { const int v = *verdict_src; *verdict_dev = v; *verdict_pin = v; }
    if (i >= n) return;
    const double u = (double)raw[i] / 4294967296.0;
    const size_t c = (size_t)(u * (double)K);
    const double f = (F[c] + (double)c) / (double)K;
    parent[i] = (f == 1.0) ? c : ((u < f) ? c : (size_t)A[c]);
}

__global__ __launch_bounds__(256) void k_widen(const uint32_t* __restrict__ raw, size_t n,
                                               unsigned long long* __restrict__ out) {
    const size_t i = (size_t)blockIdx.x * 256 + threadIdx.x;
    if (i < n) out[i] = raw[i];
}


__device__ __forceinline__ double d_recast(const abc_prior& pr, double v) {
    return (pr.kind == ABC_PRIOR_UNIF_INT) ? round(v) : v;
}
__device__ __forceinline__ bool d_valid(const abc_prior& pr, double v) {
    if (pr.kind == ABC_PRIOR_GAUSS) {
        const double u = (v - pr.a) / fabs(pr.b);
        if (u * u < 1400.0 && fabs(pr.b) < 1e10) return true;
        return (1.0 / (sqrt(2.0 * M_PI) * fabs(pr.b))) * exp(-u * u / 2.0) != 0.0;
    }
    if (pr.kind == ABC_PRIOR_UNIF_INT) return (v == round(v)) && (pr.a <= v) && (v <= pr.b);
    return (pr.a <= v) && (v <= pr.b);
}
__device__ __forceinline__ double recast_valid(const abc_prior& pr, double inv_sigma, double v, bool& ok) {
    const int kind = __builtin_amdgcn_readfirstlane(pr.kind);
    if (kind == ABC_PRIOR_GAUSS) {
        const double t = (v - pr.a) * inv_sigma;
        if (!(t * t < 1399.0 && inv_sigma != 0.0)) ok = ok && d_valid(pr, v);
        return v;
    }
    if (kind == ABC_PRIOR_UNIF_INT) v = round(v);
    ok = ok && (pr.a <= v) && (v <= pr.b);
    return v;
}
__device__ __forceinline__ double d_prior_mean(const abc_prior& pr) {
    return (pr.kind == ABC_PRIOR_GAUSS) ? pr.a : (pr.b + pr.a) / 2.0;
}

__device__ __forceinline__ void note_giveup(unsigned long long* __restrict__ g) {
    atomicAdd(g, 1ull);
    unsigned* f = (unsigned*)(size_t)g[2];
    if (f) *f = 1u;
}

constexpr unsigned MVN_MAX_TRIES = 1u << 14;

template <int PP>
__global__ __launch_bounds__(256) void k_theta_rows(const double* __restrict__ theta, size_t K, int P,
                                                    double* __restrict__ rows, const double* __restrict__ L,
                                                    double* __restrict__ Lpad) {
    __shared__ double t[PP][65];
    if (blockIdx.x == 0 && L) {
        for (int e = threadIdx.x; e < PP * PP; e += 256) {
            const int a = e % PP, b = e / PP;
            Lpad[e] = (a < P && b < P && b <= a) ? L[a + (size_t)P * b] : 0.0;
        }
    }
    const size_t k0 = (size_t)blockIdx.x * 64;
    for (int e = threadIdx.x; e < PP * 64; e += 256) {
        const int p = e >> 6, r = e & 63;
        t[p][r] = (p < P && k0 + r < K) ? theta[k0 + r + K * (size_t)p] : 0.0;
    }
    __syncthreads();
    for (int e = threadIdx.x; e < PP * 64; e += 256) {
        const int r = e / PP, p = e % PP;
        if (k0 + r < K) rows[(k0 + r) * PP + p] = t[p][r];
    }
}

template <int PP, int A0>
__device__ __forceinline__ void mv_cols4(const double* __restrict__ l, const double (&z)[4], double (&x)[PP]) {
#pragma unroll
    for (int a = A0; a < PP; a++) {
        x[a] = fma(l[a], z[0], x[a]); x[a] = fma(l[PP + a], z[1], x[a]);
        x[a] = fma(l[2 * PP + a], z[2], x[a]); x[a] = fma(l[3 * PP + a], z[3], x[a]);
    }
}
template <int PP>
__device__ __forceinline__ void mv_noise(const double* __restrict__ sL, unsigned long long gi, unsigned attempt, uint32_t k0,
                                         uint32_t k1, double (&x)[PP], int P) {
    const int nq = (P + 3) / 4;
#pragma unroll
    for (int a = 0; a < PP; a++) x[a] = 0.0;
    if constexpr (PP < 4) {
        U4 c; c.x = (uint32_t)gi; c.y = (uint32_t)(gi >> 32); c.z = attempt; c.w = 0u;
        double z[4];
        normal4(philox(c, k0, k1), z);
#pragma unroll
        for (int b = 0; b < PP; b++)
#pragma unroll
            for (int a = 0; a < PP; a++) x[a] = fma(sL[PP * b + a], z[b], x[a]);
    } else {
#pragma unroll 1
        for (int qd = 0; qd < nq; qd++) {
            U4 c; c.x = (uint32_t)gi; c.y = (uint32_t)(gi >> 32); c.z = attempt; c.w = (uint32_t)qd;
            double z[4];
            normal4(philox(c, k0, k1), z);
            const double* l = sL + PP * (4 * qd);
            if constexpr (PP >= 32) {
                const int g = (4 * qd) / (PP / 4);
                if (g == 0) mv_cols4<PP, 0>(l, z, x);
                else if (g == 1) mv_cols4<PP, PP / 4>(l, z, x);
                else if (g == 2) mv_cols4<PP, PP / 2>(l, z, x);
                else mv_cols4<PP, 3 * (PP / 4)>(l, z, x);
            } else {
                if (qd < (PP / 4 + 1) / 2) mv_cols4<PP, 0>(l, z, x);
                else mv_cols4<PP, PP / 2>(l, z, x);
            }
        }
    }
}
__device__ __forceinline__ double indep_noise(double sigma, unsigned long long gi, unsigned attempt, int p, uint32_t k0, uint32_t k1) {
    U4 c; c.x = (uint32_t)gi; c.y = (uint32_t)(gi >> 32); c.z = attempt; c.w = 0x80000000u | (uint32_t)p;
    double z[4];
    normal4(philox(c, k0, k1), z);
    return sigma * z[0];
}
template <int PP, bool MV>
__global__ __launch_bounds__(256, (MV && PP <= 16) ? 3 : (PP <= 16 ? 2 : 1)) void k_perturb(abc_rng key, const double* __restrict__ theta, size_t K, int P,
                                                 const abc_prior* __restrict__ priors,
                                                 const unsigned long long* __restrict__ parent,
                                                 unsigned long long i0, size_t n,
                                                 const double* __restrict__ L_or_dv , double* __restrict__ out,
                                                 unsigned long long* __restrict__ giveups) {
    __shared__ double sS[PP];
    __shared__ abc_prior sp[PP];
    __shared__ double sinv[PP];
    if (!MV) for (int p = threadIdx.x; p < PP; p += 256) sS[p] = (p < P) ? sqrt(L_or_dv[p]) : 0.0;
    for (int p = threadIdx.x; p < PP; p += 256) {
        abc_prior q; q.kind = ABC_PRIOR_UNIF_REAL; q.pad_ = 0; q.a = -1e300; q.b = 1e300;
        sp[p] = (p < P) ? priors[p] : q;
        sinv[p] = (p < P && priors[p].kind == ABC_PRIOR_GAUSS && fabs(priors[p].b) < 1e10 && fabs(priors[p].b) > 1e-300) ? 1.0 / fabs(priors[p].b) : 0.0;
    }
    __syncthreads();
    const size_t i = (size_t)blockIdx.x * 256 + threadIdx.x;
    if (i >= n) return;
    {
    const unsigned long long gi = i0 + i;
    const double* mrow = theta + (size_t)parent[i] * PP;
    const uint32_t k0 = key.s1 ^ 0x5bd1e995u, k1 = key.s2 ^ (key.s3 * 0x9E3779B1u);
    double x[PP];
    if (MV) {
        for (unsigned attempt = 0; attempt < MVN_MAX_TRIES; attempt++) {
            mv_noise<PP>(L_or_dv, gi, attempt, k0, k1, x, P);
            bool ok = true;
            asm volatile("" ::: "memory");
#pragma unroll
            for (int a = 0; a < PP; a += 2) {
                if (PP > 32 && a >= P) continue;
                const double2 m = *reinterpret_cast<const double2*>(mrow + a);
                x[a] = recast_valid(sp[a], sinv[a], x[a] + m.x, ok);
                x[a + 1] = recast_valid(sp[a + 1], sinv[a + 1], x[a + 1] + m.y, ok);
            }
            if (ok) break;
            if (attempt + 1 == MVN_MAX_TRIES) {
#pragma unroll
                for (int a = 0; a < PP; a++) x[a] = mrow[a];
                note_giveup(giveups);
            }
        }
    } else {
#pragma unroll
        for (int p = 0; p < PP; p++) {
            x[p] = 0.0;
            if (p < P) {
                const double m = mrow[p];
                double v = 0.0; bool ok = false;
                asm volatile("" ::: "memory");
                for (unsigned attempt = 0; attempt < 1000 && !ok; attempt++) {
                    v = d_recast(sp[p], indep_noise(sS[p], gi, attempt, p, k0, k1) + m);
                    ok = d_valid(sp[p], v);
                }
                x[p] = ok ? v : d_prior_mean(sp[p]);
                if (!ok) note_giveup(giveups);
            }
        }
    }
#pragma unroll
    for (int p = 0; p < PP; p++)
        if (p < P) __builtin_nontemporal_store(x[p], &out[i + n * (size_t)p]);
    }
}

template <int PP, bool MV>
__global__ __launch_bounds__(256) void k_perturb_stream(abc_rng key, const double* __restrict__ theta, size_t K, int P,
                                                        const abc_prior* __restrict__ priors,
                                                        const unsigned long long* __restrict__ parent,
                                                        unsigned long long i0, size_t n,
                                                        const double* __restrict__ L_or_dv, double* __restrict__ out,
                                                        unsigned long long* __restrict__ giveups) {
    extern __shared__ double smem[];
    double* sL = smem;
    abc_prior* sp = reinterpret_cast<abc_prior*>(smem + (MV ? PP * PP : PP));
    if (MV) {
        for (int e = threadIdx.x; e < PP * PP; e += 256) {
            const int a = e % PP, b = e / PP;
            sL[e] = (a < P && b < P && b <= a) ? L_or_dv[a + (size_t)P * b] : 0.0;
        }
    } else {
        for (int e = threadIdx.x; e < PP; e += 256) sL[e] = (e < P) ? sqrt(L_or_dv[e]) : 0.0;
    }
    for (int p = threadIdx.x; p < PP; p += 256) {
        abc_prior q; q.kind = ABC_PRIOR_UNIF_REAL; q.pad_ = 0; q.a = -1e300; q.b = 1e300;
        sp[p] = (p < P) ? priors[p] : q;
    }
    __syncthreads();
    const size_t i = (size_t)blockIdx.x * 256 + threadIdx.x;
    if (i >= n) return;
    const unsigned long long gi = i0 + i;
    const double* mu = theta + (size_t)parent[i] * PP;
    const uint32_t k0 = key.s1 ^ 0x5bd1e995u, k1 = key.s2 ^ (key.s3 * 0x9E3779B1u);
    if (MV) {
        bool ok = false;
        for (unsigned attempt = 0; attempt < MVN_MAX_TRIES && !ok; attempt++) {
            double x[PP];
#pragma unroll
            for (int a = 0; a < PP; a++) x[a] = 0.0;
#pragma unroll 1
            for (int qd = 0; qd < PP / 4; qd++) {
                U4 c; c.x = (uint32_t)gi; c.y = (uint32_t)(gi >> 32); c.z = attempt; c.w = (uint32_t)qd;
                double z[4];
                normal4(philox(c, k0, k1), z);
                const double* l = sL + PP * (4 * qd);
#pragma unroll
                for (int a = 0; a < PP; a++) {
                    x[a] = fma(l[a], z[0], x[a]); x[a] = fma(l[PP + a], z[1], x[a]);
                    x[a] = fma(l[2 * PP + a], z[2], x[a]); x[a] = fma(l[3 * PP + a], z[3], x[a]);
                }
            }
            ok = true;
#pragma unroll
            for (int a = 0; a < PP; a++) {
                if (a < P) {
                    const double v = d_recast(sp[a], x[a] + mu[a]);
                    out[i + n * (size_t)a] = v;
                    ok = ok && d_valid(sp[a], v);
                }
            }
        }
        if (!ok) {
            for (int p = 0; p < P; p++) out[i + n * (size_t)p] = mu[p];
            note_giveup(giveups);
        }
    } else {
        for (int p = 0; p < P; p++) {
            const double m = mu[p];
            double v = 0.0; bool ok = false;
            for (unsigned attempt = 0; attempt < 1000 && !ok; attempt++) {
                U4 c; c.x = (uint32_t)gi; c.y = (uint32_t)(gi >> 32); c.z = attempt; c.w = 0x80000000u | (uint32_t)p;
                double z[4];
                normal4(philox(c, k0, k1), z);
                v = d_recast(sp[p], sL[p] * z[0] + m);
                ok = d_valid(sp[p], v);
            }
            out[i + n * (size_t)p] = ok ? v : d_prior_mean(sp[p]);
            if (!ok) note_giveup(giveups);
        }
    }
}

__global__ __launch_bounds__(256) void k_theta_rows_gen(const double* __restrict__ theta, size_t K, int P, int PP,
                                                        double* __restrict__ rows, const double* __restrict__ L,
                                                        double* __restrict__ Lpad) {
    if (blockIdx.x == 0 && L) {
        for (size_t e = threadIdx.x; e < (size_t)PP * PP; e += 256) {
            const int a = (int)(e % PP), b = (int)(e / PP);
            Lpad[e] = (a < P && b < P && b <= a) ? L[a + (size_t)P * b] : 0.0;
        }
    }
    const size_t tot = K * (size_t)PP;
    for (size_t e = (size_t)blockIdx.x * 256 + threadIdx.x; e < tot; e += (size_t)gridDim.x * 256) {
        const size_t r = e / PP;
        const int p = (int)(e % PP);
        rows[e] = (p < P) ? theta[r + K * (size_t)p] : 0.0;
    }
}
template <bool MV>
__global__ __launch_bounds__(256) void k_perturb_gen(abc_rng key, const double* __restrict__ rows, int P, int PP,
                                                     const abc_prior* __restrict__ priors,
                                                     const unsigned long long* __restrict__ parent,
                                                     unsigned long long i0, size_t n, const double* __restrict__ L_or_dv,
                                                     double* __restrict__ out, unsigned long long* __restrict__ giveups) {
    extern __shared__ abc_prior spg[];
    for (int p = threadIdx.x; p < P; p += 256) spg[p] = priors[p];
    __syncthreads();
    const size_t i = (size_t)blockIdx.x * 256 + threadIdx.x;
    if (i >= n) return;
    const unsigned long long gi = i0 + i;
    const double* mu = rows + (size_t)parent[i] * PP;
    const uint32_t k0 = key.s1 ^ 0x5bd1e995u, k1 = key.s2 ^ (key.s3 * 0x9E3779B1u);
    if (MV) {
        bool ok = false;
        for (unsigned attempt = 0; attempt < MVN_MAX_TRIES && !ok; attempt++) {
            ok = true;
            for (int c = 0; c < PP / 64; c++) {
                double x[64];
#pragma unroll
                for (int a = 0; a < 64; a++) x[a] = 0.0;
                for (int qd = 0; qd < 16 * (c + 1); qd++) {
                    U4 cn; cn.x = (uint32_t)gi; cn.y = (uint32_t)(gi >> 32); cn.z = attempt; cn.w = (uint32_t)qd;
                    double z[4];
                    normal4(philox(cn, k0, k1), z);
                    const double* l = L_or_dv + (size_t)PP * (4 * qd) + 64 * c;
// ... 1 lines not shown
                    for (int a = 0; a < 64; a++) {
                        x[a] = fma(l[a], z[0], x[a]); x[a] = fma(l[PP + a], z[1], x[a]);
                        x[a] = fma(l[2 * (size_t)PP + a], z[2], x[a]); x[a] = fma(l[3 * (size_t)PP + a], z[3], x[a]);
                    }
                }
#pragma unroll
                for (int a = 0; a < 64; a++) {
                    const int p = 64 * c + a;
                    if (p < P) {
                        const double v = d_recast(spg[p], x[a] + mu[p]);
                        out[i + n * (size_t)p] = v;
                        ok = ok && d_valid(spg[p], v);
                    }
                }
            }
        }
        if (!ok) {
            for (int p = 0; p < P; p++) out[i + n * (size_t)p] = mu[p];
            note_giveup(giveups);
        }
    } else {
        for (int p = 0; p < P; p++) {
            const double m = mu[p], sg = sqrt(L_or_dv[p]);
            double v = 0.0; bool ok = false;
            for (unsigned attempt = 0; attempt < 1000 && !ok; attempt++) {
                v = d_recast(spg[p], indep_noise(sg, gi, attempt, p, k0, k1) + m);
                ok = d_valid(spg[p], v);
            }
            out[i + n * (size_t)p] = ok ? v : d_prior_mean(spg[p]);
            if (!ok) note_giveup(giveups);
        }
    }
}

int ensure_jump_tab(abc_ctx* ctx) {
    if (ctx->jump_tab) return ABC_OK;
    const BitMat(*tab)[3] = taus_pow2();
    std::vector<uint32_t> h(32 * 96);
    for (int k = 0; k < 32; k++)
        for (int c = 0; c < 3; c++)
            for (int i = 0; i < 32; i++) h[(size_t)k * 96 + c * 32 + i] = tab[k + RUN_LOG2][c].col[i];
    ABC_HIP(ctx, hipMalloc((void**)&ctx->jump_tab, h.size() * sizeof(uint32_t)));
    ABC_HIP(ctx, hipMemcpy(ctx->jump_tab, h.data(), h.size() * sizeof(uint32_t), hipMemcpyHostToDevice));
    return ABC_OK;
}

int taus_stream(abc_ctx* ctx, abc_rng base, size_t n, uint32_t* out, hipStream_t st = nullptr) {
    ABC_TRY(ensure_jump_tab(ctx));
    const size_t threads = (n + RUN - 1) / RUN;
    const unsigned bs = (threads <= (size_t)256 * 64 * 4) ? 64u : 256u;
    hipLaunchKernelGGL(k_taus_stream, dim3((unsigned)((threads + bs - 1) / bs)), dim3(bs), 0, st ? st : ctx->stream, base, n,
                       ctx->jump_tab, out);
    ABC_HIP(ctx, hipGetLastError());
    return ABC_OK;
}


}

int abc_uniform_alias(abc_ctx* ctx, size_t K) {
    if (K == 0 || K > 0xffffffffull) ABC_FAIL(ctx, ABC_ERR_INVALID, "resample: K = %zu", K);
    if (ctx->ualias_K == K) return ABC_OK;
    ctx->ualias_K = 0;
    if (ctx->ualias_cap < K) {
        ABC_HIP(ctx, hipStreamSynchronize(ctx->stream));
        if (ctx->ualias_F) { (void)hipFree(ctx->ualias_F); ctx->ualias_F = nullptr; }
        if (ctx->ualias_pin) { (void)hipHostFree(ctx->ualias_pin); ctx->ualias_pin = nullptr; }
        ctx->ualias_cap = 0;
        ABC_HIP(ctx, hipMalloc((void**)&ctx->ualias_F, K * (sizeof(double) + sizeof(uint32_t))));
        ABC_HIP(ctx, hipHostMalloc((void**)&ctx->ualias_pin, K * (sizeof(double) + sizeof(uint32_t)), hipHostMallocDefault));
        ctx->ualias_cap = K;
    }
    ABC_TRY(abc_pin_reserve(ctx, K * (sizeof(double) * 2 + sizeof(uint32_t) * 2) + 2 * sizeof(uint32_t)));
    double* hw = (double*)ctx->pin;
    double* hE = hw + K;
    uint32_t* hS = (uint32_t*)(hE + K);
    uint32_t* hB = hS + K + 1;
    double* hF = (double*)ctx->ualias_pin;
    uint32_t* hA = (uint32_t*)(hF + K);
    const double v = 1.0 / (double)K;
    for (size_t k = 0; k < K; k++) hw[k] = v;
    const auto t0 = std::chrono::steady_clock::now();
    abc_alias_preproc(K, hw, hF, hA, hE, hS, hB, false);
    if (ctx->timing) {
        ctx->stage_host_ms[ST_ALIAS_HOST] += std::chrono::duration<double, std::milli>(std::chrono::steady_clock::now() - t0).count();
        ctx->stage_cnt[ST_ALIAS_HOST] += 1;
    }
    ctx->ualias_A = (uint32_t*)(ctx->ualias_F + K);
    ABC_HIP(ctx, hipMemcpyAsync(ctx->ualias_F, hF, K * (sizeof(double) + sizeof(uint32_t)), hipMemcpyHostToDevice, ctx->stream));
    ctx->ualias_K = K;
    return ABC_OK;
}

static int launch_seeds(abc_ctx* ctx, const abc_rng* rng, uint64_t i0, size_t n, uint64_t* seeds, uint64_t seed_stream_offset,
                        hipStream_t st);

int abc_side_fork(abc_ctx* ctx) {
    if (!ctx->side) {
        ABC_HIP(ctx, hipStreamCreateWithFlags(&ctx->side, hipStreamNonBlocking));
        ABC_HIP(ctx, hipEventCreateWithFlags(&ctx->ev_fork, abc_xstream_event_flags()));
        ABC_HIP(ctx, hipEventCreateWithFlags(&ctx->ev_side, abc_xstream_event_flags()));
    }
    if (hipStreamQuery(ctx->stream) != hipSuccess) {
        (void)hipGetLastError();
        ABC_HIP(ctx, hipEventRecord(ctx->ev_fork, ctx->stream));
        ABC_HIP(ctx, hipStreamWaitEvent(ctx->side, ctx->ev_fork, 0));
    }
    ctx->side_forked = true;
    return ABC_OK;
}

int abc_rng_streams_early(abc_ctx* ctx, const abc_rng* rng, uint64_t i0, size_t n, uint64_t* seeds, uint64_t seed_stream_offset,
                          uint32_t** raw_out, uint64_t* parent_uniform, size_t K_uniform) {
    *raw_out = nullptr;
    if (n == 0) return ABC_OK;
    uint32_t* raw = (uint32_t*)abc_ws_alloc(ctx, n * sizeof(uint32_t));
    if (!raw) ABC_FAIL(ctx, ABC_ERR_NOMEM, "resample: workspace exhausted");
    ABC_TRY(ensure_jump_tab(ctx));
    if (!ctx->side_forked) ABC_TRY(abc_side_fork(ctx));
    abc_rng base = *rng;
    taus2_jump(&base, i0);
    ABC_TRY(taus_stream(ctx, base, n, raw, ctx->side));
    if (parent_uniform && ctx->ualias_K == K_uniform && K_uniform) {
        hipLaunchKernelGGL(k_alias_draw, dim3((unsigned)((n + 255) / 256)), dim3(256), 0, ctx->side, raw, n, ctx->ualias_F,
                           ctx->ualias_A, K_uniform, (unsigned long long*)parent_uniform);
        ABC_HIP(ctx, hipGetLastError());
    }
    if (seeds) ABC_TRY(launch_seeds(ctx, rng, i0, n, seeds, seed_stream_offset, ctx->side));
    ABC_HIP(ctx, hipEventRecord(ctx->ev_side, ctx->side));
    *raw_out = raw;
    return ABC_OK;
}

int abc_rng_seeds_early(abc_ctx* ctx, const abc_rng* rng, uint64_t i0, size_t n, uint64_t* seeds, uint64_t seed_stream_offset) {
    if (n == 0 || !seeds) return ABC_OK;
    if (!ctx->side_forked) ABC_TRY(abc_side_fork(ctx));
    ABC_TRY(launch_seeds(ctx, rng, i0, n, seeds, seed_stream_offset, ctx->side));
    ABC_HIP(ctx, hipEventRecord(ctx->ev_side, ctx->side));
    return ABC_OK;
}

int abc_weights_prev_early(abc_ctx* ctx, size_t P, size_t kn_max, const double* theta_prev, size_t Kp, const double* w_prev,
                           const double* dv_prev, abc_wprev* out) {
    if (!ctx->side_forked) ABC_TRY(abc_side_fork(ctx));
    if (!ctx->ev_prev) ABC_HIP(ctx, hipEventCreateWithFlags(&ctx->ev_prev, abc_xstream_event_flags()));
    ABC_TRY(launch_weights_prev(ctx, P, kn_max, theta_prev, Kp, w_prev, dv_prev, out, ctx->side));
    ABC_HIP(ctx, hipEventRecord(ctx->ev_prev, ctx->side));
    return ABC_OK;
}

int launch_resample(abc_ctx* ctx, const abc_rng* rng, const double* w, size_t K, uint64_t i0, size_t n,
                    uint64_t* parent, int (*while_host_builds)(void*), void* hook_arg, bool uniform_weights,
                    const uint32_t* raw_ready, bool weights_on_host, const volatile int* abort_flag, bool parents_ready,
                    int* alias_check_deferred) {
    if (alias_check_deferred) *alias_check_deferred = 0;
    bool wait_side = raw_ready != nullptr;
    if (n == 0) return ABC_OK;
    if (K == 0 || K > 0xffffffffull) ABC_FAIL(ctx, ABC_ERR_INVALID, "resample: K = %zu", K);
    if (uniform_weights) {
        ABC_TRY(abc_uniform_alias(ctx, K));
        uint32_t* raw = const_cast<uint32_t*>(raw_ready);
        if (!raw) raw = (uint32_t*)abc_ws_alloc(ctx, n * sizeof(uint32_t));
        if (!raw) ABC_FAIL(ctx, ABC_ERR_NOMEM, "resample: workspace exhausted");
        abc_rng base = *rng;
        taus2_jump(&base, i0);
        StageTimer tm(ctx, ST_RESAMPLE);
        if (raw_ready) ABC_HIP(ctx, hipStreamWaitEvent(ctx->stream, ctx->ev_side, 0));
        else ABC_TRY(taus_stream(ctx, base, n, raw));
        if (while_host_builds) ABC_TRY(while_host_builds(hook_arg));
        if (!(parents_ready && raw_ready)) {
            hipLaunchKernelGGL(k_alias_draw, dim3((unsigned)((n + 255) / 256)), dim3(256), 0, ctx->stream, raw, n, ctx->ualias_F,
                               ctx->ualias_A, K, (unsigned long long*)parent);
            ABC_HIP(ctx, hipGetLastError());
        }
        return ABC_OK;
    }
    if (ctx->alias_K < K) {
        ABC_HIP(ctx, hipStreamSynchronize(ctx->stream));
        if (ctx->alias_F) { (void)hipFree(ctx->alias_F); ctx->alias_F = nullptr; ctx->alias_A = nullptr; }
        ABC_HIP(ctx, hipMalloc((void**)&ctx->alias_F, K * (sizeof(double) + sizeof(uint32_t))));
        ctx->alias_K = K;
    }
    ctx->alias_A = (uint32_t*)(ctx->alias_F + K);
    if (ctx->alias_mode == ABC_ALIAS_DEVICE && K >= ABC_ALIAS_DEV_MIN_K && K <= ABC_ALIAS_DEV_MAX_K && ctx->ws_off + abc_alias_dev_need(K) <= ctx->ws_bytes) {
        if (!ctx->alias_fail_dev) ABC_HIP(ctx, hipMalloc((void**)&ctx->alias_fail_dev, sizeof(int)));
        int* fail_pin = &ctx->status_pin->alias_fail;
        *fail_pin = 0;
        const int* verdict = nullptr;
        uint32_t* raw = const_cast<uint32_t*>(raw_ready);
        if (!raw) raw = (uint32_t*)abc_ws_alloc(ctx, n * sizeof(uint32_t));
        if (!raw) ABC_FAIL(ctx, ABC_ERR_NOMEM, "resample: workspace exhausted");
        abc_rng base = *rng;
        taus2_jump(&base, i0);
        if (raw_ready) {
            if (!ctx->side_early_waited) ABC_HIP(ctx, hipStreamWaitEvent(ctx->stream, ctx->ev_side, 0));
        } else {
            StageTimer tm(ctx, ST_RESAMPLE);
            ABC_TRY(taus_stream(ctx, base, n, raw));
        }
        {
            StageTimer tm(ctx, ST_ALIAS_HOST);
            ABC_TRY(launch_alias_build_dev(ctx, w, K, ctx->alias_F, ctx->alias_A, ctx->alias_fail_dev, fail_pin, &verdict));
        }
        ctx->alias_dev_builds++;
        if (while_host_builds) ABC_TRY(while_host_builds(hook_arg));
        {
            StageTimer tm(ctx, ST_RESAMPLE);
            hipLaunchKernelGGL(k_alias_draw, dim3((unsigned)((n + 255) / 256)), dim3(256), 0, ctx->stream, raw, n, ctx->alias_F,
                               ctx->alias_A, K, (unsigned long long*)parent, verdict, ctx->alias_fail_dev, fail_pin);
            ABC_HIP(ctx, hipGetLastError());
        }
        if (alias_check_deferred) { *alias_check_deferred = 1; return ABC_OK; }
        ABC_HIP(ctx, hipStreamSynchronize(ctx->stream));
        if (!*fail_pin) return ABC_OK;
        ctx->alias_dev_fallbacks++;
        while_host_builds = nullptr;
        raw_ready = raw;
        wait_side = false;
        weights_on_host = false;
    }
    ABC_TRY(abc_pin_reserve(ctx, abc_alias_pin_bytes(K)));
    double* hw = (double*)ctx->pin;
    double* hF = hw + K;
    uint32_t* hA = (uint32_t*)(hF + K);
    double* hE = (double*)(((uintptr_t)(hA + K) + 7) & ~(uintptr_t)7);
    uint32_t* hS = (uint32_t*)(hE + K);
    uint32_t* hB = hS + K + 1;
    if (!weights_on_host)
        ABC_HIP(ctx, hipMemcpyAsync(hw, w, K * sizeof(double), hipMemcpyDeviceToHost, ctx->stream));
    if (!ctx->ev_copy) ABC_HIP(ctx, hipEventCreateWithFlags(&ctx->ev_copy, hipEventDisableTiming));
    ABC_HIP(ctx, hipEventRecord(ctx->ev_copy, ctx->stream));
    uint32_t* raw = const_cast<uint32_t*>(raw_ready);
    if (!raw) raw = (uint32_t*)abc_ws_alloc(ctx, n * sizeof(uint32_t));
    if (!raw) ABC_FAIL(ctx, ABC_ERR_NOMEM, "resample: workspace exhausted");
    abc_rng base = *rng;
    taus2_jump(&base, i0);
    if (raw_ready) {
        if (wait_side && !ctx->side_early_waited) ABC_HIP(ctx, hipStreamWaitEvent(ctx->stream, ctx->ev_side, 0));
    } else {
        StageTimer tm(ctx, ST_RESAMPLE);
        ABC_TRY(taus_stream(ctx, base, n, raw));
    }
    if (while_host_builds) ABC_TRY(while_host_builds(hook_arg));
    ABC_HIP(ctx, hipEventSynchronize(ctx->ev_copy));
    if (abort_flag && *abort_flag) return ABC_INTERNAL_RETRY;
    {
        const auto t0 = std::chrono::steady_clock::now();
        abc_alias_preproc(K, hw, hF, hA, hE, hS, hB, false);
        if (ctx->timing) {
            ctx->stage_host_ms[ST_ALIAS_HOST] += std::chrono::duration<double, std::milli>(std::chrono::steady_clock::now() - t0).count();
            ctx->stage_cnt[ST_ALIAS_HOST] += 1;
        }
    }
    StageTimer tm(ctx, ST_RESAMPLE);
    ABC_HIP(ctx, hipMemcpyAsync(ctx->alias_F, hF, K * (sizeof(double) + sizeof(uint32_t)), hipMemcpyHostToDevice, ctx->stream));
    hipLaunchKernelGGL(k_alias_draw, dim3((unsigned)((n + 255) / 256)), dim3(256), 0, ctx->stream, raw, n, ctx->alias_F,
                       ctx->alias_A, K, (unsigned long long*)parent);
    ABC_HIP(ctx, hipGetLastError());
    return ABC_OK;
}

static int launch_theta_rows(abc_ctx* ctx, const double* theta, size_t K, size_t P, int PP, double* rows, const double* L,
                             double* Lpad) {
    const unsigned grid = (unsigned)((K + 63) / 64);
    if (PP > 64) {
        size_t gb = (K * (size_t)PP + 255) / 256;
        if (gb > 4096) gb = 4096;
        hipLaunchKernelGGL(k_theta_rows_gen, dim3((unsigned)gb), dim3(256), 0, ctx->stream, theta, K, (int)P, PP, rows, L, Lpad);
        ABC_HIP(ctx, hipGetLastError());
        return ABC_OK;
    }
    switch (PP) {
        case 2: hipLaunchKernelGGL((k_theta_rows<2>), dim3(grid), dim3(256), 0, ctx->stream, theta, K, (int)P, rows, L, Lpad); break;
        case 4: hipLaunchKernelGGL((k_theta_rows<4>), dim3(grid), dim3(256), 0, ctx->stream, theta, K, (int)P, rows, L, Lpad); break;
        case 8: hipLaunchKernelGGL((k_theta_rows<8>), dim3(grid), dim3(256), 0, ctx->stream, theta, K, (int)P, rows, L, Lpad); break;
        case 16: hipLaunchKernelGGL((k_theta_rows<16>), dim3(grid), dim3(256), 0, ctx->stream, theta, K, (int)P, rows, L, Lpad); break;
        case 32: hipLaunchKernelGGL((k_theta_rows<32>), dim3(grid), dim3(256), 0, ctx->stream, theta, K, (int)P, rows, L, Lpad); break;
        default: hipLaunchKernelGGL((k_theta_rows<64>), dim3(grid), dim3(256), 0, ctx->stream, theta, K, (int)P, rows, L, Lpad); break;
    }
    ABC_HIP(ctx, hipGetLastError());
    return ABC_OK;
}
static int launch_seeds(abc_ctx* ctx, const abc_rng* rng, uint64_t i0, size_t n, uint64_t* seeds, uint64_t seed_stream_offset,
                        hipStream_t st) {
    uint32_t* raw = (uint32_t*)abc_ws_alloc(ctx, n * sizeof(uint32_t));
    if (!raw) ABC_FAIL(ctx, ABC_ERR_NOMEM, "perturb: workspace exhausted");
    abc_rng base = *rng;
    taus2_jump(&base, seed_stream_offset + i0);
    ABC_TRY(taus_stream(ctx, base, n, raw, st));
    hipLaunchKernelGGL(k_widen, dim3((unsigned)((n + 255) / 256)), dim3(256), 0, st ? st : ctx->stream, raw, n, (unsigned long long*)seeds);
    ABC_HIP(ctx, hipGetLastError());
    return ABC_OK;
}
int launch_perturb_prepare(abc_ctx* ctx, const abc_rng* rng, const double* theta, size_t K, size_t P, uint64_t i0, size_t n,
                           uint64_t* seeds, uint64_t seed_stream_offset, abc_perturb_prep* prep, int multivariate,
                           const double* L_or_dv) {
    if (n == 0) { prep->rows = nullptr; prep->Lpad = nullptr; return ABC_OK; }
    const int PP = abc_perturb_pp(P);
    StageTimer tm(ctx, ST_PERTURB);
    if (!prep->rows) {
        double* rows = (double*)abc_ws_alloc(ctx, K * (size_t)PP * sizeof(double));
        double* Lpad = (multivariate && L_or_dv) ? (double*)abc_ws_alloc(ctx, (size_t)PP * PP * sizeof(double)) : nullptr;
        if (!rows || (multivariate && L_or_dv && !Lpad)) ABC_FAIL(ctx, ABC_ERR_NOMEM, "perturb: workspace exhausted");
        ABC_TRY(launch_theta_rows(ctx, theta, K, P, PP, rows, Lpad ? L_or_dv : nullptr, Lpad));
        prep->rows = rows;
        prep->Lpad = Lpad;
    }
    if (seeds && !prep->seeds_done) { ABC_TRY(launch_seeds(ctx, rng, i0, n, seeds, seed_stream_offset, nullptr)); prep->seeds_done = 1; }
    return ABC_OK;
}

int abc_giveups_ensure(abc_ctx* ctx) {
    if (ctx->giveups_dev) return ABC_OK;
    ABC_HIP(ctx, hipMalloc((void**)&ctx->giveups_dev, 3 * sizeof(unsigned long long)));
    const unsigned long long init[3] = {0ull, 0ull, (unsigned long long)(size_t)&ctx->status_pin->giveup_flag};
    ABC_HIP(ctx, hipMemcpy(ctx->giveups_dev, init, sizeof(init), hipMemcpyHostToDevice));
    return ABC_OK;
}

int launch_perturb(abc_ctx* ctx, const abc_rng* rng, const double* theta, size_t K, size_t P, const abc_prior* priors,
                   const uint64_t* parent, uint64_t i0, size_t n, int multivariate, const double* L_or_dv, double* out,
                   uint64_t* seeds, uint64_t seed_stream_offset, const abc_perturb_prep* prep) {
    if (n == 0) return ABC_OK;
    int PP = 2;
    while (PP < (int)P) PP *= 2;
    if (P > 64) PP = (int)((P + 63) / 64 * 64);
    ABC_TRY(abc_giveups_ensure(ctx));
    StageTimer tm(ctx, ST_PERTURB);
    const unsigned blocks = (unsigned)((n + 255) / 256);
    double* rows = (prep && prep->rows) ? prep->rows : (double*)abc_ws_alloc(ctx, K * (size_t)PP * sizeof(double));
    if (!rows) ABC_FAIL(ctx, ABC_ERR_NOMEM, "perturb: workspace exhausted");
    const double* Lpad = (prep && prep->rows) ? prep->Lpad : nullptr;
    if (!(prep && prep->rows)) {
        const bool need_lp = multivariate != 0;
        double* lp = need_lp ? (double*)abc_ws_alloc(ctx, (size_t)PP * PP * sizeof(double)) : nullptr;
        if (need_lp && !lp) ABC_FAIL(ctx, ABC_ERR_NOMEM, "perturb: workspace exhausted");
        ABC_TRY(launch_theta_rows(ctx, theta, K, P, PP, rows, lp ? L_or_dv : nullptr, lp));
        Lpad = lp;
    }
    theta = rows;
    if (multivariate && !Lpad) ABC_FAIL(ctx, ABC_ERR_INVALID, "perturb: the padded factor was not prepared");
    if (PP > 64) {
        const size_t lds = P * sizeof(abc_prior);
        if (multivariate)
            hipLaunchKernelGGL((k_perturb_gen<true>), dim3(blocks), dim3(256), lds, ctx->stream, *rng, theta, (int)P, PP, priors,
                               (const unsigned long long*)parent, (unsigned long long)i0, n, Lpad, out, ctx->giveups_dev);
        else
            hipLaunchKernelGGL((k_perturb_gen<false>), dim3(blocks), dim3(256), lds, ctx->stream, *rng, theta, (int)P, PP, priors,
                               (const unsigned long long*)parent, (unsigned long long)i0, n, L_or_dv, out, ctx->giveups_dev);
        ABC_HIP(ctx, hipGetLastError());
        if (seeds && !(prep && prep->seeds_done)) ABC_TRY(launch_seeds(ctx, rng, i0, n, seeds, seed_stream_offset, nullptr));
        return ABC_OK;
    }
#define LAUNCH_PT(PPV)                                                                                                 \
    do {                                                                                                               \
        if (multivariate)                                                                                              \
            hipLaunchKernelGGL((k_perturb<PPV, true>), dim3(blocks), dim3(256), 0, ctx->stream, *rng, theta, K, (int)P, \
                               priors, (const unsigned long long*)parent, (unsigned long long)i0, n, Lpad, out,       \
                               ctx->giveups_dev);                                                                     \
        else                                                                                                           \
            hipLaunchKernelGGL((k_perturb<PPV, false>), dim3(blocks), dim3(256), 0, ctx->stream, *rng, theta, K, (int)P, \
                               priors, (const unsigned long long*)parent, (unsigned long long)i0, n, L_or_dv, out,    \
                               ctx->giveups_dev);                                                                     \
    } while (0)
    switch (PP) {
        case 2: LAUNCH_PT(2); break;
        case 4: LAUNCH_PT(4); break;
        case 8: LAUNCH_PT(8); break;
        case 16: LAUNCH_PT(16); break;
        case 32: LAUNCH_PT(32); break;
        default:
            if (multivariate) {
                LAUNCH_PT(64);
            } else {
                const size_t lds = 64 * sizeof(double) + 64 * sizeof(abc_prior);
                hipLaunchKernelGGL((k_perturb_stream<64, false>), dim3(blocks), dim3(256), lds, ctx->stream, *rng, theta, K,
                                   (int)P, priors, (const unsigned long long*)parent, (unsigned long long)i0, n, L_or_dv, out,
                                   ctx->giveups_dev);
            }
            break;
    }
#undef LAUNCH_PT
    ABC_HIP(ctx, hipGetLastError());
    if (seeds && !(prep && prep->seeds_done)) ABC_TRY(launch_seeds(ctx, rng, i0, n, seeds, seed_stream_offset, nullptr));
    return ABC_OK;
}

int abc_moments_on_side(abc_ctx* ctx, const double* theta, size_t K, size_t P, bool multivariate, double* L_io, double* dv,
                        int* spd_dev, const double* model_hdr, bool theta_ev_bound, const char* who, abc_side_moments* m) {
    m->L = m->stats = nullptr;
    if (multivariate) {
        m->L = L_io ? L_io : (double*)abc_ws_alloc(ctx, P * P * 8);
        if (!m->L) ABC_FAIL(ctx, ABC_ERR_NOMEM, "%s: workspace exhausted", who);
    }
    const int PPr = abc_perturb_pp(P);
    abc_status_block* pin = ctx->status_pin;
    m->out = {dv, m->L, spd_dev, nullptr, nullptr, model_hdr, pin->model_hdr, m->L ? &pin->spd : nullptr};
    pin->model_hdr[0] = 0.0; pin->spd = 0;
    m->out.rows = (double*)abc_ws_alloc(ctx, K * (size_t)PPr * sizeof(double));
    if (m->L) m->out.Lpad = (double*)abc_ws_alloc(ctx, (size_t)PPr * PPr * sizeof(double));
    if (!m->out.rows || (m->L && !m->out.Lpad)) ABC_FAIL(ctx, ABC_ERR_NOMEM, "%s: workspace exhausted", who);
    if (!theta_ev_bound) ABC_HIP(ctx, hipEventRecord(ctx->ev_theta, ctx->stream));
    ABC_HIP(ctx, hipStreamWaitEvent(ctx->side, ctx->ev_theta, 0));
    {
        StreamScope on_side(ctx, ctx->side);
        ABC_TRY(launch_theta_stats(ctx, theta, K, P, &m->stats));
        ABC_TRY(launch_post_tail(ctx, theta, K, P, m->stats, &m->out));
    }
    ABC_HIP(ctx, hipEventRecord(ctx->ev_moments, ctx->side));
    return ABC_OK;
}

int abc_normalize_for_resample(abc_ctx* ctx, double* w, size_t K, size_t Nn, const double* sumsq, bool* w_on_host) {
    double* mirror = nullptr;
    const bool alias_on_device = ctx->alias_mode == ABC_ALIAS_DEVICE && K >= ABC_ALIAS_DEV_MIN_K && K <= ABC_ALIAS_DEV_MAX_K;
    if (Nn && !alias_on_device) {
        ABC_TRY(abc_pin_reserve(ctx, abc_alias_pin_bytes(K)));
        mirror = (double*)ctx->pin;
    }
    ABC_TRY(launch_normalize_l2(ctx, w, K, mirror, sumsq));
    *w_on_host = mirror != nullptr;
    return ABC_OK;
}

int abc_prep_hook(void* a) {
    abc_prep_arg* q = (abc_prep_arg*)a;
    int fused_done = 0;
    if (q->moments) {
        StageTimer tm(q->ctx, ST_GATHER_DV);
        double* st = nullptr;
        ABC_TRY(launch_theta_stats(q->ctx, q->theta, q->K, q->P, &st));
        q->theta_stats = st;
        abc_theta_fused f = {q->dv, q->L, q->spd_dev, nullptr, nullptr, q->model_hdr, q->hdr_pin, q->spd_pin};
        if (q->ctx->noise_mode != ABC_NOISE_REFERENCE_STREAM) {
            const int PP = abc_perturb_pp(q->P);
            f.rows = (double*)abc_ws_alloc(q->ctx, q->K * (size_t)PP * sizeof(double));
            if (q->L) f.Lpad = (double*)abc_ws_alloc(q->ctx, (size_t)PP * PP * sizeof(double));
            if (!f.rows || (q->L && !f.Lpad)) ABC_FAIL(q->ctx, ABC_ERR_NOMEM, "generation: workspace exhausted");
        }
        ABC_TRY(launch_post_tail(q->ctx, q->theta, q->K, q->P, st, &f));
        q->prep->rows = f.rows;
        q->prep->Lpad = f.Lpad;
        fused_done = 1;
    }
    if (q->L && !fused_done) {
        if (q->theta_stats) {
            StageTimer tm(q->ctx, ST_MVN);
            ABC_TRY(launch_mvn_from_stats(q->ctx, q->theta_stats, q->P, q->L, q->spd_dev));
        } else {
            ABC_TRY(launch_mvn_setup(q->ctx, q->theta, q->K, q->P, q->L, nullptr, q->spd_dev));
        }
    }
    if (q->ctx->noise_mode == ABC_NOISE_REFERENCE_STREAM) return ABC_OK;
    return launch_perturb_prepare(q->ctx, q->rng, q->theta, q->K, q->P, q->i0, q->Nn, q->seeds, q->seed_off, q->prep,
                                  q->L ? 1 : 0, q->L ? q->L : q->dv);
}

int abc_alias_repair(abc_ctx* ctx, const abc_rng* rng_entry, const double* w, size_t K, uint64_t i0, size_t Nn, uint64_t seed_off,
                     uint64_t* parent, const double* theta, size_t P, const abc_prior* priors, int multivariate, const double* L_or_dv,
                     double* next, abc_perturb_prep* prep, bool giveups_to_snapshot) {
    ctx->alias_dev_fallbacks++;
    const int mode = ctx->alias_mode;
    ctx->alias_mode = ABC_ALIAS_HOST;
    const int rc = launch_resample(ctx, rng_entry, w, K, i0, Nn, parent);
    ctx->alias_mode = mode;
    ABC_TRY(rc);
    prep->seeds_done = 1;
    if (giveups_to_snapshot && ctx->giveups_dev)
        ABC_HIP(ctx, hipMemcpyAsync(ctx->giveups_dev, ctx->giveups_dev + 1, sizeof(unsigned long long), hipMemcpyDeviceToDevice, ctx->stream));
    ABC_TRY(launch_perturb(ctx, rng_entry, theta, K, P, priors, parent, i0, Nn, multivariate, L_or_dv, next, nullptr, seed_off, prep));
    ABC_HIP(ctx, hipStreamSynchronize(ctx->stream));
    return ABC_OK;
}

int launch_perturb_reference(abc_ctx* ctx, abc_rng* rng_after_draws, const double* theta, size_t K, size_t P,
                             const abc_prior* priors, const uint64_t* parent, size_t n, int multivariate, const double* L_or_dv,
                             double* out, uint64_t* seeds) {
    if (n == 0) return ABC_OK;
    StageTimer tm(ctx, ST_PERTURB);
    std::vector<double> hth(K * P), hl(multivariate ? P * P : P), hout(n * P);
    std::vector<uint64_t> hpar(n), hseeds(seeds ? n : 0);
    std::vector<abc_prior> hpr(P);
    ABC_HIP(ctx, hipMemcpyAsync(hth.data(), theta, hth.size() * 8, hipMemcpyDeviceToHost, ctx->stream));
    ABC_HIP(ctx, hipMemcpyAsync(hl.data(), L_or_dv, hl.size() * 8, hipMemcpyDeviceToHost, ctx->stream));
    ABC_HIP(ctx, hipMemcpyAsync(hpar.data(), parent, n * 8, hipMemcpyDeviceToHost, ctx->stream));
    ABC_HIP(ctx, hipMemcpyAsync(hpr.data(), priors, P * sizeof(abc_prior), hipMemcpyDeviceToHost, ctx->stream));
    ABC_HIP(ctx, hipStreamSynchronize(ctx->stream));
    const auto t0 = std::chrono::steady_clock::now();
    if (multivariate) {
        for (size_t a = 0; a < P; a++)
            for (size_t b = a + 1; b < P; b++) hl[a + P * b] = 0.0;
        ctx->giveups_host += abc_ref_perturb_mvn(rng_after_draws, n, K, P, hth.data(), hpar.data(), hl.data(), hpr.data(),
                                                 MVN_MAX_TRIES, hout.data());
    } else {
        ctx->giveups_host += abc_ref_perturb_indep(rng_after_draws, n, K, P, hth.data(), hpar.data(), hl.data(), hpr.data(),
                                                   hout.data());
    }
    if (seeds) abc_ref_seeds(rng_after_draws, n, hseeds.data());
    ctx->stage_host_ms[ST_PERTURB] += std::chrono::duration<double, std::milli>(std::chrono::steady_clock::now() - t0).count();
    ABC_HIP(ctx, hipMemcpyAsync(out, hout.data(), hout.size() * 8, hipMemcpyHostToDevice, ctx->stream));
    if (seeds) ABC_HIP(ctx, hipMemcpyAsync(seeds, hseeds.data(), n * 8, hipMemcpyHostToDevice, ctx->stream));
    ABC_HIP(ctx, hipStreamSynchronize(ctx->stream));
    return ABC_OK;
}
```

abcsmc_amd/csrc/sharded.hip:

```cpp
#include <dlfcn.h>
#include <rccl/rccl.h>

#include <cmath>
#include <condition_variable>
#include <mutex>
#include <thread>
#include <vector>

#include "abc_internal.h"
#include <hip/hip_ext.h>

namespace {

struct Rccl {
    void* h = nullptr;
    decltype(&ncclGetUniqueId) GetUniqueId = nullptr;
    decltype(&ncclCommInitRank) CommInitRank = nullptr;
    decltype(&ncclCommInitAll) CommInitAll = nullptr;
    decltype(&ncclCommDestroy) CommDestroy = nullptr;
    decltype(&ncclCommAbort) CommAbort = nullptr;
    decltype(&ncclAllReduce) AllReduce = nullptr;
    decltype(&ncclAllGather) AllGather = nullptr;
    decltype(&ncclBroadcast) Broadcast = nullptr;
    decltype(&ncclGetErrorString) GetErrorString = nullptr;
// ... 525 lines not shown
        ABC_TRY(xbuf_reserve(ctx, (size_t)(W + 1) * R.rec_bytes + tot * 40 + 4096));
        char* rec_mine = ctx->xbuf;
        char* rec_all = rec_mine + R.rec_bytes;
        double* cand_dist = (double*)(rec_all + (size_t)W * R.rec_bytes);
        uint64_t* cand_idx = (uint64_t*)(cand_dist + tot);
        double* mrg_dist = (double*)(cand_idx + tot);
        uint64_t* mrg_idx = (uint64_t*)(mrg_dist + tot);
        uint64_t* mrg_src = mrg_idx + tot;
        int* ds_fail = (int*)abc_ws_alloc(ctx, sizeof(int));
        if (!ds_fail) ABC_FAIL(ctx, ABC_ERR_NOMEM, "sharded generation: workspace exhausted");
        const size_t ls_n = ls_cap < n ? ls_cap : n;
        if (ls_n) ABC_TRY(launch_select_smallest(ctx, dist, n, ls_n, row0, (uint64_t*)R.idx(rec_mine, 0), (double*)R.dist(rec_mine, 0), true));
        const bool bins_deferred = ls_n && ctx->sel_bins_ran && ctx->sel_fail_dev && !ctx->sel_force_radix;
        ctx->sel_bins_ran = false;
        if (ls_n < ls_cap)
            hipLaunchKernelGGL(k_pad_tail, dim3((unsigned)((ls_cap - ls_n + 255) / 256)), dim3(256), 0, ctx->stream, (double*)R.dist(rec_mine, 0),
                               (unsigned long long*)R.idx(rec_mine, 0), ls_n, ls_cap);
        hipLaunchKernelGGL(k_ls_header, dim3(1), dim3(64), 0, ctx->stream, (unsigned long long*)R.hdr(rec_mine, 0), (unsigned long long)ls_n,
                           (unsigned long long)n, bins_deferred ? (const int*)ctx->sel_fail_dev : (const int*)nullptr);
        if (ls_n) ABC_TRY(launch_gather_rows(ctx, io->Y, n, n, P, (const uint64_t*)R.idx(rec_mine, 0), ls_n, row0, (double*)R.rows(rec_mine, 0), ls_cap));
        ABC_TRY(comm_all_gather(ctx, rec_mine, rec_all, R.rec_bytes));
        pfail_early = &ctx->status_pin->gather_sel_fail;
        *pfail_early = 0;
        ds_fail_dev = ds_fail;
        hipLaunchKernelGGL(k_ls_unpack, dim3((unsigned)((tot + 255) / 256)), dim3(256), 0, ctx->stream, (const char*)rec_all, R, W, cand_dist,
                           (unsigned long long*)cand_idx, ds_fail, pfail_early);
        ABC_HIP(ctx, hipGetLastError());
        ABC_TRY(launch_merge_runs(ctx, cand_dist, cand_idx, W, ls_cap, mrg_dist, mrg_idx, mrg_src));
        hipLaunchKernelGGL(k_ls_check, dim3(1), dim3(64), 0, ctx->stream, (const char*)rec_all, R, W, (const double*)mrg_dist, K, ds_fail, pfail_early);
        if (moments_planned) {
            hipExtLaunchKernelGGL(k_ds_place, dim3((unsigned)((K * (P + 1) + 255) / 256)), dim3(256), 0, ctx->stream, nullptr, ctx->ev_theta, 0,
                                  (const char*)rec_all, R, (const double*)mrg_dist, (const unsigned long long*)mrg_src, K, (const int*)ds_fail,
                                  (unsigned long long*)io->idx, io->dist, theta);
            theta_ev_bound = true;
        } else
            hipLaunchKernelGGL(k_ds_place, dim3((unsigned)((K * (P + 1) + 255) / 256)), dim3(256), 0, ctx->stream, (const char*)rec_all, R,
                               (const double*)mrg_dist, (const unsigned long long*)mrg_src, K, (const int*)ds_fail,
                               (unsigned long long*)io->idx, io->dist, theta);
        ABC_HIP(ctx, hipGetLastError());
    } else {
        ABC_TRY(launch_select_begin(ctx, K, sel_state, sel_hist));
        for (int p = 0; p < 6; p++) {
            ABC_TRY(launch_select_hist(ctx, dist, n, sel_state, p, sel_hist));
            ABC_TRY(comm_all_reduce(ctx, sel_hist, 2048, ABC_DT_I32));
            ABC_TRY(launch_select_pick(ctx, sel_state, p, sel_hist, K));
        }
        ABC_TRY(launch_select_count(ctx, dist, n, sel_state, counts));
        ABC_TRY(comm_all_gather(ctx, counts, counts + 2, 2 * sizeof(long long)));
        long long* hc = (long long*)ctx->pin;
        ABC_HIP(ctx, hipMemcpyAsync(hc, counts + 2, (size_t)(2 * W) * sizeof(long long), hipMemcpyDeviceToHost, ctx->stream));
        ABC_HIP(ctx, hipStreamSynchronize(ctx->stream));
        long long remaining = (long long)K, maxw = 0, my_less = 0, my_take = 0;
        for (int q = 0; q < W; q++) remaining -= hc[2 * q];
        if (remaining < 0) ABC_FAIL(ctx, ABC_ERR_COMM, "distributed selection: %lld keys below the K-th", (long long)K - remaining);
        for (int q = 0; q < W; q++) {
            const long long tq = hc[2 * q + 1] < remaining ? hc[2 * q + 1] : remaining;
            remaining -= tq;
            const long long nwq = hc[2 * q] + tq;
            if (nwq > maxw) maxw = nwq;
            if (q == r) { my_less = hc[2 * q]; my_take = tq; }
        }
        if (remaining != 0) ABC_FAIL(ctx, ABC_ERR_COMM, "distributed selection: %lld winners missing", remaining);
        const size_t mw = (size_t)maxw, nw = (size_t)(my_less + my_take), tot = (size_t)W * mw;
        const size_t xb = (2 * mw + 5 * tot) * 8 + (mw + tot) * P * 8 + 4096;
        ABC_TRY(xbuf_reserve(ctx, xb));
        char* xp = ctx->xbuf;
        auto take = [&](size_t bytes) { char* p0 = xp; xp += abc_align(bytes, 256); return p0; };
        uint64_t* loc_idx = (uint64_t*)take(mw * 8);
        double* loc_dist = (double*)take(mw * 8);
        uint64_t* cand_idx = (uint64_t*)take(tot * 8);
        double* cand_dist = (double*)take(tot * 8);
        uint64_t* mrg_idx = (uint64_t*)take(tot * 8);
        double* mrg_dist = (double*)take(tot * 8);
        uint64_t* mrg_src = (uint64_t*)take(tot * 8);
        double* rows_mine = (double*)take(mw * P * 8);
        double* rows_all = (double*)take(tot * P * 8);
        if ((size_t)(xp - ctx->xbuf) > ctx->xbuf_bytes) ABC_FAIL(ctx, ABC_ERR_NOMEM, "sharded generation: exchange buffer");
        ABC_TRY(launch_select_compact(ctx, dist, n, sel_state, (uint64_t)my_less, (uint64_t)my_take, row0, loc_idx, loc_dist));
        if (nw > 1) ABC_TRY(launch_sort_pairs(ctx, loc_dist, loc_idx, nw));
        if (nw < mw)
            hipLaunchKernelGGL(k_pad_tail, dim3((unsigned)((mw - nw + 255) / 256)), dim3(256), 0, ctx->stream, loc_dist,
                               (unsigned long long*)loc_idx, nw, mw);
        ABC_TRY(comm_all_gather(ctx, loc_idx, cand_idx, mw * 8));
        ABC_TRY(comm_all_gather(ctx, loc_dist, cand_dist, mw * 8));
        ABC_TRY(launch_merge_runs(ctx, cand_dist, cand_idx, W, mw, mrg_dist, mrg_idx, mrg_src));
        ABC_HIP(ctx, hipMemcpyAsync(io->idx, mrg_idx, K * 8, hipMemcpyDeviceToDevice, ctx->stream));
        if (io->dist) ABC_HIP(ctx, hipMemcpyAsync(io->dist, mrg_dist, K * 8, hipMemcpyDeviceToDevice, ctx->stream));
        if (nw) ABC_TRY(launch_gather_rows(ctx, io->Y, n, n, P, loc_idx, nw, row0, rows_mine, mw));
        ABC_TRY(comm_all_gather(ctx, rows_mine, rows_all, mw * P * 8));
        hipLaunchKernelGGL(k_place_rows, dim3((unsigned)((K * P + 255) / 256)), dim3(256), 0, ctx->stream, rows_all,
                           (const unsigned long long*)mrg_src, K, (int)P, mw, theta);
        ABC_HIP(ctx, hipGetLastError());
    }

    auto repeat_with_radix = [&]() -> int {
        ABC_HIP(ctx, hipStreamSynchronize(ctx->stream));
        if (ctx->side) ABC_HIP(ctx, hipStreamSynchronize(ctx->side));
        *rng = rng_entry;
        ctx->sel_force_radix = true;
        const int rc = sharded_core(ctx, cfg, io, rng, ncomp_host);
        ctx->sel_force_radix = false;
        return rc;
    };
    double* dv = io->dv ? io->dv : (double*)abc_ws_alloc(ctx, P * 8);
    double* theta_stats = nullptr;
    abc_side_moments side = {};
    bool moments_on_side = false, status_early = false;
    if (moments_planned) {
        ABC_TRY(abc_moments_on_side(ctx, theta, K, P, cfg->multivariate != 0, io->L, dv, spd_dev, model, theta_ev_bound, "sharded generation", &side));
        theta_stats = side.stats;
        moments_on_side = status_early = true;
    } else if (P <= 64 && K >= 2) {
        StageTimer tm(ctx, ST_GATHER_DV);
        ABC_TRY(launch_theta_stats(ctx, theta, K, P, &theta_stats));
        ABC_TRY(launch_dv_from_stats(ctx, theta_stats, P, dv));
    } else {
        ABC_TRY(launch_doubled_variance(ctx, theta, K, P, dv));
    }
    bool w_on_host = false;
    if (Kp == 0 || !io->theta_prev) {
        ABC_TRY(launch_fill(ctx, io->w, K, 1.0 / (double)K));
    } else {
        if (wprev.ready) ABC_HIP(ctx, hipStreamWaitEvent(ctx->stream, ctx->ev_prev, 0));
        const double* sumsq = nullptr;
        if (W == 1) {
            ABC_TRY(launch_weights_raw(ctx, io->priors, theta, K, P, 0, K, io->theta_prev, Kp, io->w_prev, io->dv_prev, io->w, &wprev, &sumsq));
        } else {
            if (kn) ABC_TRY(launch_weights_raw(ctx, io->priors, theta, K, P, k0, kn, io->theta_prev, Kp, io->w_prev, io->dv_prev, w_mine, &wprev));
            ABC_TRY(comm_all_gather(ctx, w_mine, w_slices, kmax * 8));
            hipLaunchKernelGGL(k_unpad_slices, dim3((unsigned)((K + 255) / 256)), dim3(256), 0, ctx->stream, w_slices, K, W, kmax, io->w);
            ABC_HIP(ctx, hipGetLastError());
        }
        ABC_TRY(abc_normalize_for_resample(ctx, io->w, K, Nn, sumsq, &w_on_host));
    }

    int spd = 0;
    bool have_spd = false;
    int alias_deferred = 0;
    uint64_t* parent_used = nullptr;
    double* L_used = nullptr;
    abc_perturb_prep prep_used = {nullptr, 0, nullptr};
    if (Nn) {
        uint64_t* parent = io->parent ? io->parent : (uint64_t*)abc_ws_alloc(ctx, Nn * 8);
        if (!parent) ABC_FAIL(ctx, ABC_ERR_NOMEM, "sharded generation: workspace exhausted");
        double* L = nullptr;
        if (cfg->multivariate) {
            L = side.L ? side.L : (io->L ? io->L : (double*)abc_ws_alloc(ctx, P * P * 8));
            have_spd = true;
        }
        abc_perturb_prep prep = {side.out.rows, io->seeds ? 1 : 0, side.out.Lpad};
        if (moments_on_side) ABC_HIP(ctx, hipStreamWaitEvent(ctx->stream, ctx->ev_moments, 0));
        abc_prep_arg pa = {ctx, rng, theta, theta_stats, K, P, Nn, cfg->next0, cfg->Nnext_total, io->seeds, &prep, moments_on_side ? nullptr : L,
                           spd_dev, dv, false, nullptr, nullptr, nullptr};
        {
            const int rc = launch_resample(ctx, rng, io->w, K, cfg->next0, Nn, parent, abc_prep_hook, &pa, uniform_w, raw_early, w_on_host,
                                           (ds_fail_dev && !uniform_w) ? pfail_early : nullptr, false, &alias_deferred);
            if (rc == ABC_INTERNAL_RETRY) return repeat_with_radix();
            ABC_TRY(rc);
        }
        ABC_TRY(launch_perturb(ctx, rng, theta, K, P, io->priors, parent, cfg->next0, Nn, cfg->multivariate,
                               cfg->multivariate ? L : dv, io->next, io->seeds, cfg->Nnext_total, &prep));
        parent_used = parent; L_used = L; prep_used = prep;
    } else if (cfg->multivariate && io->L) {
        have_spd = true;
        if (theta_stats) ABC_TRY(launch_mvn_from_stats(ctx, theta_stats, P, io->L, spd_dev));
        else ABC_TRY(launch_mvn_setup(ctx, theta, K, P, io->L, nullptr, spd_dev));
    }
    taus2_jump(rng, 2 * (uint64_t)cfg->Nnext_total);
    {
        double* hdr = ctx->status_pin->model_hdr;
        int* pspd = &ctx->status_pin->spd;
        if (!status_early) {
            hdr[0] = 0.0; *pspd = 0;
            ABC_HIP(ctx, hipMemcpyAsync(hdr, model, 4 * sizeof(double), hipMemcpyDeviceToHost, ctx->stream));
            if (have_spd) ABC_HIP(ctx, hipMemcpyAsync(pspd, spd_dev, sizeof(int), hipMemcpyDeviceToHost, ctx->stream));
        }
        ABC_HIP(ctx, hipStreamSynchronize(ctx->stream));
        if (ncomp_host) *ncomp_host = (int32_t)hdr[0];
        spd = *pspd;
        if (ds_fail_dev && pfail_early && *pfail_early) return repeat_with_radix();
        if (alias_deferred && *(volatile int*)&ctx->status_pin->alias_fail && parent_used) {
            ABC_TRY(abc_alias_repair(ctx, &rng_entry, io->w, K, cfg->next0, Nn, cfg->Nnext_total, parent_used, theta, P, io->priors,
                                     cfg->multivariate, cfg->multivariate ? L_used : dv, io->next, &prep_used, false));
        }
    }
    {
        volatile unsigned* pgaveup = &ctx->status_pin->giveup_flag;
        if (Nn && *pgaveup && ctx->giveups_dev) {
            unsigned long long now = 0;
            ABC_HIP(ctx, hipMemcpyAsync(&now, ctx->giveups_dev, sizeof(now), hipMemcpyDeviceToHost, ctx->stream));
            ABC_HIP(ctx, hipStreamSynchronize(ctx->stream));
            ctx->giveups_dev_known = now;
        }
        const unsigned long long gv = ctx->giveups_dev_known + ctx->giveups_host, before = ctx->giveups_seen;
        ctx->giveups_seen = gv;
        ctx->giveups_last_call = (Nn && gv > before) ? gv - before : 0ull;
    }
    if (spd) ABC_FAIL(ctx, ABC_ERR_NOT_SPD, "covariance of the selected particles is not positive definite");
    return ABC_OK;
}

extern "C" int abc_generation_multi(abc_ctx* const* ctxs, int ndev, const abc_generation_cfg* cfg, const abc_generation_io* h,
                                    abc_rng* rng, int32_t* ncomp) {
    if (!ctxs || ndev < 1 || !ctxs[0]) return ABC_ERR_INVALID;
    abc_ctx* c0 = ctxs[0];
    if (!cfg || !h || !h->X || !h->Y || !h->obs || !h->priors || !h->idx || !h->w || !rng)
        ABC_FAIL(c0, ABC_ERR_INVALID, "multi-GPU generation: null argument");
    for (int d = 0; d < ndev; d++)
        if (!ctxs[d] || (ndev > 1 && (ctxs[d]->comm_kind != 1 || ctxs[d]->comm_world != ndev || ctxs[d]->comm_rank != d)))
            ABC_FAIL(c0, ABC_ERR_INVALID, "multi-GPU generation: context %d is not rank %d of an %d-rank communicator", d, d, ndev);
    const size_t N = cfg->N, M = cfg->M, P = cfg->P, K = cfg->K, Kp = cfg->Kp, Nn = cfg->Nnext;
    if (!N || !M || !P || !K || K > N) ABC_FAIL(c0, ABC_ERR_INVALID, "multi-GPU generation: bad sizes");
    if (Kp && (!h->theta_prev || !h->w_prev || !h->dv_prev)) ABC_FAIL(c0, ABC_ERR_INVALID, "multi-GPU generation: previous set missing");
    std::vector<int> rcs((size_t)ndev, ABC_OK);
    std::vector<int32_t> ncs((size_t)ndev, 0);
    std::vector<abc_rng> rngs((size_t)ndev, *rng);
    std::mutex mu;
    std::condition_variable cv;
    int arrived = 0, any_failed = 0;
    auto agree = [&](int my_status) -> bool {
        std::unique_lock<std::mutex> lk(mu);
        if (my_status != ABC_OK) any_failed = 1;
        if (++arrived == ndev) cv.notify_all();
        else cv.wait(lk, [&] { return arrived == ndev; });
        return any_failed == 0;
    };
    auto worker = [&](int d) {
        abc_ctx* ctx = ctxs[d];
        auto fail = [&](int rc) { rcs[(size_t)d] = rc; };
        if (hipSetDevice(ctx->device) != hipSuccess) { snprintf(ctx->err, sizeof(ctx->err), "hipSetDevice failed"); (void)agree(ABC_ERR_HIP); return fail(ABC_ERR_HIP); }
        auto lo = [&](size_t tot, int q) { return tot / (size_t)ndev * (size_t)q + ((size_t)q < tot % (size_t)ndev ? (size_t)q : tot % (size_t)ndev); };
        const size_t r0 = lo(N, d), n = lo(N, d + 1) - r0, i0 = lo(Nn, d), nn = lo(Nn, d + 1) - i0;
        std::vector<void*> bufs;
        auto dmalloc = [&](size_t bytes) -> void* {
            void* p = nullptr;
            if (hipMalloc(&p, bytes ? bytes : 8) != hipSuccess) return nullptr;
            bufs.push_back(p);
            return p;
        };
        auto cleanup = [&] { (void)hipStreamSynchronize(ctx->stream); for (void* p : bufs) (void)hipFree(p); };
        double* dX = (double*)dmalloc(n * M * 8);
        double* dY = (double*)dmalloc(n * P * 8);
        double* dobs = (double*)dmalloc(M * 8);
        abc_prior* dpri = (abc_prior*)dmalloc(P * sizeof(abc_prior));
        double *dtp = nullptr, *dwp = nullptr, *ddvp = nullptr;
        if (Kp) { dtp = (double*)dmalloc(Kp * P * 8); dwp = (double*)dmalloc(Kp * 8); ddvp = (double*)dmalloc(P * 8); }
        uint64_t* didx = (uint64_t*)dmalloc(K * 8);
        double* ddist = (double*)dmalloc(K * 8);
        double* dth = (double*)dmalloc(K * P * 8);
        double* dw = (double*)dmalloc(K * 8);
        double* ddv = (double*)dmalloc(P * 8);
        double* dL = (double*)dmalloc(P * P * 8);
        double* dnext = (double*)dmalloc(nn * P * 8);
        uint64_t* dpar = (uint64_t*)dmalloc(nn * 8);
        uint64_t* dseed = (uint64_t*)dmalloc(nn * 8);
        if (!dX || !dY || !dobs || !dpri || (Kp && (!dtp || !dwp || !ddvp)) || !didx || !ddist || !dth || !dw || !ddv || !dL || !dnext ||
            !dpar || !dseed) {
            snprintf(ctx->err, sizeof(ctx->err), "multi-GPU generation: device allocation failed");
            (void)agree(ABC_ERR_NOMEM);
            cleanup();
            return fail(ABC_ERR_NOMEM);
        }
        hipStream_t st = ctx->stream;
        bool ok = true;
        auto H = [&](hipError_t e) { if (e != hipSuccess && ok) { ok = false; snprintf(ctx->err, sizeof(ctx->err), "multi-GPU generation: %s", hipGetErrorString(e)); } };
        if (n) {
            H(hipMemcpy2DAsync(dX, n * 8, h->X + r0, N * 8, n * 8, M, hipMemcpyHostToDevice, st));
            H(hipMemcpy2DAsync(dY, n * 8, h->Y + r0, N * 8, n * 8, P, hipMemcpyHostToDevice, st));
        }
        H(hipMemcpyAsync(dobs, h->obs, M * 8, hipMemcpyHostToDevice, st));
        H(hipMemcpyAsync(dpri, h->priors, P * sizeof(abc_prior), hipMemcpyHostToDevice, st));
        if (Kp) {
            H(hipMemcpyAsync(dtp, h->theta_prev, Kp * P * 8, hipMemcpyHostToDevice, st));
            H(hipMemcpyAsync(dwp, h->w_prev, Kp * 8, hipMemcpyHostToDevice, st));
            H(hipMemcpyAsync(ddvp, h->dv_prev, P * 8, hipMemcpyHostToDevice, st));
        }
        if (!agree(ok ? ABC_OK : ABC_ERR_HIP)) {
            cleanup();
            if (ok) snprintf(ctx->err, sizeof(ctx->err), "multi-GPU generation: skipped, the set-up of another device failed");
            return fail(ok ? ABC_ERR_COMM : ABC_ERR_HIP);
        }
        abc_sharded_cfg sc;
        memset(&sc, 0, sizeof(sc));
        sc.n_local = n; sc.row0 = r0; sc.N_total = N; sc.M = M; sc.P = P; sc.K = K; sc.Kp = Kp;
        sc.nnext_local = nn; sc.next0 = i0; sc.Nnext_total = Nn; sc.train_frac = cfg->train_frac;
        sc.max_comp = cfg->max_comp; sc.rule = cfg->rule; sc.multivariate = cfg->multivariate;
        abc_generation_io io;
        memset(&io, 0, sizeof(io));
        io.X = dX; io.Y = dY; io.obs = dobs; io.priors = dpri; io.theta_prev = dtp; io.w_prev = dwp; io.dv_prev = ddvp;
        io.idx = didx; io.dist = ddist; io.theta = dth; io.w = dw; io.dv = ddv; io.L = dL; io.next = dnext; io.parent = dpar; io.seeds = dseed;
        const int rc = abc_generation_sharded_dev(ctx, &sc, &io, &rngs[(size_t)d], &ncs[(size_t)d]);
        if (rc != ABC_OK) { cleanup(); return fail(rc); }
        if (d == 0) {
            H(hipMemcpyAsync(h->idx, didx, K * 8, hipMemcpyDeviceToHost, st));
            if (h->dist) H(hipMemcpyAsync(h->dist, ddist, K * 8, hipMemcpyDeviceToHost, st));
            if (h->theta) H(hipMemcpyAsync(h->theta, dth, K * P * 8, hipMemcpyDeviceToHost, st));
            H(hipMemcpyAsync(h->w, dw, K * 8, hipMemcpyDeviceToHost, st));
            if (h->dv) H(hipMemcpyAsync(h->dv, ddv, P * 8, hipMemcpyDeviceToHost, st));
            if (h->L && cfg->multivariate) H(hipMemcpyAsync(h->L, dL, P * P * 8, hipMemcpyDeviceToHost, st));
        }
        if (nn) {
            if (h->next) H(hipMemcpy2DAsync(h->next + i0, Nn * 8, dnext, nn * 8, nn * 8, P, hipMemcpyDeviceToHost, st));
            if (h->parent) H(hipMemcpyAsync(h->parent + i0, dpar, nn * 8, hipMemcpyDeviceToHost, st));
            if (h->seeds) H(hipMemcpyAsync(h->seeds + i0, dseed, nn * 8, hipMemcpyDeviceToHost, st));
        }
        H(hipStreamSynchronize(st));
        cleanup();
        if (!ok) return fail(ABC_ERR_HIP);
    };
    if (ndev == 1) worker(0);
    else {
        std::vector<std::thread> th;
        for (int d = 0; d < ndev; d++) th.emplace_back(worker, d);
        for (auto& t : th) t.join();
// ... 11 lines not shown
```

Before: 374.0 million particles/s.

## Fuse alias draw into perturb kernel and use wave-shuffle block scans

Defers the alias-table draw from resample and folds it into the perturb kernel. The multivariate path does the cell lookup early and resolves the parent row after the first noise block, so the parent load latency hides behind the noise math. This removes one kernel launch and the parent write-then-read round trip, though each perturb thread now does extra table loads. It also replaces the shared-memory Hillis-Steele block prefix sums in the alias builder with wave shuffles, and skips identity compositions in the RMap scans.

After: 373.6 million particles/s. About the same (-0.1%).

```diff
diff --git a/abcsmc_amd/csrc/abc_internal.h b/abcsmc_amd/csrc/abc_internal.h
--- a/abcsmc_amd/csrc/abc_internal.h
+++ b/abcsmc_amd/csrc/abc_internal.h
@@ -381,10 +381,15 @@
 static inline size_t abc_alias_pin_bytes(size_t K) { return K * (sizeof(double) * 3 + sizeof(uint32_t) * 3) + 2 * sizeof(uint32_t) + 16; }
 int launch_mvn_setup(abc_ctx*, const double* theta, size_t K, size_t P, double* L, int* status_host,
                      int* status_dev);
+struct abc_draw_deferred {
+    const uint32_t* raw; const double* F; const uint32_t* A; size_t K;
+    const int* verdict_src; int* verdict_dev; int* verdict_pin;
+};
 int launch_resample(abc_ctx*, const abc_rng* rng, const double* w, size_t K, uint64_t i0, size_t n,
                     uint64_t* parent, int (*while_host_builds)(void*) = nullptr, void* hook_arg = nullptr,
                     bool uniform_weights = false, const uint32_t* raw_ready = nullptr, bool weights_on_host = false,
-                    const volatile int* abort_flag = nullptr, bool parents_ready = false, int* alias_check_deferred = nullptr);
+                    const volatile int* abort_flag = nullptr, bool parents_ready = false, int* alias_check_deferred = nullptr,
+                    abc_draw_deferred* draw_deferred = nullptr);
 int abc_rng_streams_early(abc_ctx* ctx, const abc_rng* rng, uint64_t i0, size_t n, uint64_t* seeds, uint64_t seed_stream_offset,
                           uint32_t** raw, uint64_t* parent_uniform = nullptr, size_t K_uniform = 0);
 int abc_rng_seeds_early(abc_ctx* ctx, const abc_rng* rng, uint64_t i0, size_t n, uint64_t* seeds, uint64_t seed_stream_offset);
@@ -402,7 +407,7 @@
 int launch_perturb(abc_ctx*, const abc_rng* rng, const double* theta, size_t K, size_t P,
                    const abc_prior* priors, const uint64_t* parent, uint64_t i0, size_t n,
                    int multivariate, const double* L_or_dv, double* out, uint64_t* seeds,
-                   uint64_t seed_stream_offset, const abc_perturb_prep* prep = nullptr);
+                   uint64_t seed_stream_offset, const abc_perturb_prep* prep = nullptr, const abc_draw_deferred* draw = nullptr);
 
 struct abc_side_moments { abc_theta_fused out; double* stats; double* L; };
 int abc_moments_on_side(abc_ctx* ctx, const double* theta, size_t K, size_t P, bool multivariate, double* L_io, double* dv,
diff --git a/abcsmc_amd/csrc/alias_dev.hip b/abcsmc_amd/csrc/alias_dev.hip
--- a/abcsmc_amd/csrc/alias_dev.hip
+++ b/abcsmc_amd/csrc/alias_dev.hip
@@ -99,17 +99,18 @@
     if (lane == 0) exw = rmap_identity();
     if (lane == 63) buf[0][wave] = inc;
     __syncthreads();
-    RMap before = rmap_identity();
-    for (int w = 0; w < wave; w++) before = compose(before, buf[0][w]);
-    __syncthreads();
+    RMap before = buf[0][0];
+    for (int w = 1; w < wave; w++) before = compose(before, buf[0][w]);
+    __syncthreads();
+    if (wave == 0) { *excl = exw; return inc; }
     *excl = compose(before, exw);
     return compose(before, inc);
 }
 __device__ __forceinline__ RMap prefix_of_blocks(const RMap* __restrict__ agg, int nb, RMap (*buf)[AL_T]) {
     const int t = threadIdx.x;
     const int per = (nb + AL_T - 1) / AL_T;
-    RMap m = rmap_identity();
-    for (int j = 0; j < per; j++) { const int b = t * per + j; if (b < nb) m = compose(m, agg[b]); }
+    RMap m = (t * per < nb) ? agg[t * per] : rmap_identity();
+    for (int j = 1; j < per; j++) { const int b = t * per + j; if (b < nb) m = compose(m, agg[b]); }
     RMap ex;
     (void)block_scan_maps(m, buf, &ex);
     __shared__ RMap s_tot;
@@ -157,11 +158,16 @@
     }
 }
 
-__device__ __forceinline__ void approx_prefix(const double* __restrict__ bsum, int nblk, int b, double* sm, double* before, double* all) {
+__device__ __forceinline__ void approx_prefix(const double* __restrict__ bsum, int nblk, int b, double* sm , double* before, double* all) {
     double pb = 0.0, pa = 0.0;
     for (int j = threadIdx.x; j < nblk; j += AL_T) { const double v = bsum[j]; pa += v; if (j < b) pb += v; }
-    *before = block_sum_d(pb, sm);
-    *all = block_sum_d(pa, sm);
+#pragma unroll
+    for (int o = 32; o >= 1; o >>= 1) { pb += __shfl_xor(pb, o, 64); pa += __shfl_xor(pa, o, 64); }
+    __syncthreads();
+    if ((threadIdx.x & 63) == 0) { sm[threadIdx.x >> 6] = pb; sm[4 + (threadIdx.x >> 6)] = pa; }
+    __syncthreads();
+    *before = (sm[0] + sm[1]) + (sm[2] + sm[3]);
+    *all = (sm[4] + sm[5]) + (sm[6] + sm[7]);
 }
 
 struct SumCtx { double before, all; int e0; };
@@ -177,25 +183,27 @@
     return rne_map(k, c, sticky);
 }
 __device__ __forceinline__ double block_excl_prefix_d(double mine, double* sd ) {
-    const int t = threadIdx.x;
-    sd[t] = mine;
-    __syncthreads();
-    for (int step = 1; step < AL_T; step <<= 1) {
-        const double a = (t >= step) ? sd[t - step] : 0.0;
-        __syncthreads();
-        sd[t] += a;
-        __syncthreads();
-    }
-    const double ex = t ? sd[t - 1] : 0.0;
-    __syncthreads();
-    return ex;
+    const int lane = threadIdx.x & 63, wave = threadIdx.x >> 6;
+    double inc = mine;
+#pragma unroll
+    for (int d = 1; d < 64; d <<= 1) {
+        const double up = __shfl_up(inc, d, 64);
+        if (lane >= d) inc += up;
+    }
+    double ex = __shfl_up(inc, 1, 64);
+    if (lane == 0) ex = 0.0;
+    if (lane == 63) sd[wave] = inc;
+    __syncthreads();
+    double before = 0.0;
+    for (int w = 0; w < wave; w++) before += sd[w];
+    return before + ex;
 }
 
 __global__ __launch_bounds__(AL_T) void k_al_sum_reduce(const double* __restrict__ w, size_t K, const double* __restrict__ bsum, int nblk,
                                                         RMap* __restrict__ agg, RMap* __restrict__ tpre, AlHead* __restrict__ head) {
     __shared__ RMap buf[2][AL_T];
-    __shared__ double sd[AL_T];
-    __shared__ double sm[4];
+    __shared__ double sd[4];
+    __shared__ double sm[8];
     double before, all;
     approx_prefix(bsum, nblk, blockIdx.x, sm, &before, &all);
     int etot;
@@ -207,9 +215,10 @@
 #pragma unroll
     for (int j = 0; j < AL_I; j++) { x[j] = (base + j < K) ? w[base + j] : 0.0; ts += x[j]; }
     double run = before + block_excl_prefix_d(ts, sd);
-    RMap m = rmap_identity();
-#pragma unroll
-    for (int j = 0; j < AL_I; j++) { run += x[j]; m = compose(m, sum_map(x[j], run, e0, head)); }
+    run += x[0];
+    RMap m = sum_map(x[0], run, e0, head);
+#pragma unroll
+    for (int j = 1; j < AL_I; j++) { run += x[j]; m = compose(m, sum_map(x[j], run, e0, head)); }
     RMap ex;
     const RMap inc = block_scan_maps(m, buf, &ex);
     tpre[(size_t)blockIdx.x * AL_T + threadIdx.x] = ex;
@@ -220,8 +229,8 @@
 __global__ __launch_bounds__(AL_T) void k_al_sum_apply(const double* __restrict__ w, size_t K, const double* __restrict__ bsum, int nblk,
                                                        const RMap* __restrict__ agg, const RMap* __restrict__ tpre, AlHead* __restrict__ head) {
     __shared__ RMap buf[2][AL_T];
-    __shared__ double sd[AL_T];
-    __shared__ double sm[4];
+    __shared__ double sd[4];
+    __shared__ double sm[8];
     double before, all;
     approx_prefix(bsum, nblk, blockIdx.x, sm, &before, &all);
     int etot;
@@ -481,9 +490,9 @@
     StepRec rec[AL_I];
 #pragma unroll
     for (int j = 0; j < AL_I; j++) if (base + j < n) rec[j] = a.step[base + j];
-    RMap m = rmap_identity();
-#pragma unroll
-    for (int j = 0; j < AL_I; j++) if (base + j < n) m = compose(m, serve_map(rec[j], MEAN));
+    RMap m = (base < n) ? serve_map(rec[0], MEAN) : rmap_identity();
+#pragma unroll
+    for (int j = 1; j < AL_I; j++) if (base + j < n) m = compose(m, serve_map(rec[j], MEAN));
     RMap ex;
     const RMap inc = block_scan_maps(m, buf, &ex);
     tpre[(size_t)blockIdx.x * AL_T + threadIdx.x] = ex;
diff --git a/abcsmc_amd/csrc/api.hip b/abcsmc_amd/csrc/api.hip
--- a/abcsmc_amd/csrc/api.hip
+++ b/abcsmc_amd/csrc/api.hip
@@ -1095,10 +1095,12 @@
             pa.model_hdr = simple ? nullptr : model; pa.hdr_pin = hdr_pin; pa.spd_pin = L ? spd_pin : nullptr;
             status_early = true;
         }
+        abc_draw_deferred draw = {};
         {
             const int rc = launch_resample(ctx, rng, io->w, K, 0, Nn, parent, abc_prep_hook, &pa, uniform_w, raw_early, w_on_host,
                                            bins_deferred ? pfail_early : nullptr, parent_early != nullptr,
-                                           ctx->noise_mode == ABC_NOISE_REFERENCE_STREAM ? nullptr : &alias_deferred);
+                                           ctx->noise_mode == ABC_NOISE_REFERENCE_STREAM ? nullptr : &alias_deferred,
+                                           ctx->noise_mode == ABC_NOISE_REFERENCE_STREAM ? nullptr : &draw);
             if (rc == ABC_INTERNAL_RETRY) return repeat_with_radix();
             ABC_TRY(rc);
         }
@@ -1108,7 +1110,7 @@
                                              cfg->multivariate ? L : dv, io->next, io->seeds));
         } else {
             ABC_TRY(launch_perturb(ctx, rng, theta, K, P, io->priors, parent, 0, Nn, cfg->multivariate,
-                                   cfg->multivariate ? L : dv, io->next, io->seeds, Nn, &prep));
+                                   cfg->multivariate ? L : dv, io->next, io->seeds, Nn, &prep, &draw));
             parent_used = parent; L_used = L; prep_used = prep;
             taus2_jump(rng, 2 * (uint64_t)Nn);
         }
@@ -1374,12 +1376,14 @@
     uint64_t* dpar = s.dev<uint64_t>(n);
     uint64_t* dseed = seeds ? s.dev<uint64_t>(n) : nullptr;
     if (!dw || !dth || !dpr || !dl || !dout || !dpar) ABC_FAIL(ctx, ABC_ERR_NOMEM, "sample: workspace exhausted");
-    ABC_TRY(launch_resample(ctx, rng, dw, K, 0, n, dpar));
+    abc_draw_deferred draw = {};
+    ABC_TRY(launch_resample(ctx, rng, dw, K, 0, n, dpar, nullptr, nullptr, false, nullptr, false, nullptr, false, nullptr,
+                            ctx->noise_mode == ABC_NOISE_REFERENCE_STREAM ? nullptr : &draw));
     if (ctx->noise_mode == ABC_NOISE_REFERENCE_STREAM) {
         taus2_jump(rng, (uint64_t)n);
         ABC_TRY(launch_perturb_reference(ctx, rng, dth, K, P, dpr, dpar, n, multivariate, dl, dout, dseed));
     } else {
-        ABC_TRY(launch_perturb(ctx, rng, dth, K, P, dpr, dpar, 0, n, multivariate, dl, dout, dseed, n));
+        ABC_TRY(launch_perturb(ctx, rng, dth, K, P, dpr, dpar, 0, n, multivariate, dl, dout, dseed, n, nullptr, &draw));
         taus2_jump(rng, seeds ? 2 * (uint64_t)n : (uint64_t)n);
     }
     s.down(out, dout, n * P);
diff --git a/abcsmc_amd/csrc/resample.hip b/abcsmc_amd/csrc/resample.hip
--- a/abcsmc_amd/csrc/resample.hip
+++ b/abcsmc_amd/csrc/resample.hip
@@ -93,18 +93,31 @@
     }
 }
 
+__device__ __forceinline__ size_t alias_cell(uint32_t r, size_t K, double* u) {
+    *u = (double)r / 4294967296.0;
+    return (size_t)(*u * (double)K);
+}
+__device__ __forceinline__ size_t alias_choose(double u, size_t c, double Fc, uint32_t Ac, size_t K) {
+    const double f = (Fc + (double)c) / (double)K;
+    return (f == 1.0) ? c : ((u < f) ? c : (size_t)Ac);
+}
+__device__ __forceinline__ size_t alias_pick(uint32_t r, const double* __restrict__ F, const uint32_t* __restrict__ A, size_t K) {
+    double u;
+    const size_t c = alias_cell(r, K, &u);
+    return alias_choose(u, c, F[c], A[c], K);
+}
+__device__ __forceinline__ void publish_verdict(const int* __restrict__ src, int* __restrict__ dev, int* __restrict__ pin) {
+    const int v = *src; *dev = v; *pin = v;
+}
 __global__ __launch_bounds__(256) void k_alias_draw(const uint32_t* __restrict__ raw, size_t n,
                                                     const double* __restrict__ F, const uint32_t* __restrict__ A,
                                                     size_t K, unsigned long long* __restrict__ parent,
                                                     const int* __restrict__ verdict_src = nullptr, int* __restrict__ verdict_dev = nullptr,
                                                     int* __restrict__ verdict_pin = nullptr) {
     const size_t i = (size_t)blockIdx.x * 256 + threadIdx.x;
-    if (i == 0 && verdict_src) { const int v = *verdict_src; *verdict_dev = v; *verdict_pin = v; }
+    if (i == 0 && verdict_src) publish_verdict(verdict_src, verdict_dev, verdict_pin);
     if (i >= n) return;
-    const double u = (double)raw[i] / 4294967296.0;
-    const size_t c = (size_t)(u * (double)K);
-    const double f = (F[c] + (double)c) / (double)K;
-    parent[i] = (f == 1.0) ? c : ((u < f) ? c : (size_t)A[c]);
+    parent[i] = alias_pick(raw[i], F, A, K);
 }
 
 __global__ __launch_bounds__(256) void k_widen(const uint32_t* __restrict__ raw, size_t n,
@@ -180,9 +193,10 @@
         x[a] = fma(l[2 * PP + a], z[2], x[a]); x[a] = fma(l[3 * PP + a], z[3], x[a]);
     }
 }
-template <int PP>
+struct NoHook { __device__ __forceinline__ void operator()() const {} };
+template <int PP, typename Hook = NoHook>
 __device__ __forceinline__ void mv_noise(const double* __restrict__ sL, unsigned long long gi, unsigned attempt, uint32_t k0,
-                                         uint32_t k1, double (&x)[PP], int P) {
+                                         uint32_t k1, double (&x)[PP], int P, Hook after_first = Hook()) {
     const int nq = (P + 3) / 4;
 #pragma unroll
     for (int a = 0; a < PP; a++) x[a] = 0.0;
@@ -194,6 +208,7 @@
         for (int b = 0; b < PP; b++)
 #pragma unroll
             for (int a = 0; a < PP; a++) x[a] = fma(sL[PP * b + a], z[b], x[a]);
+        after_first();
     } else {
 #pragma unroll 1
         for (int qd = 0; qd < nq; qd++) {
@@ -211,6 +226,7 @@
                 if (qd < (PP / 4 + 1) / 2) mv_cols4<PP, 0>(l, z, x);
                 else mv_cols4<PP, PP / 2>(l, z, x);
             }
+            if (qd == 0) after_first();
         }
     }
 }
@@ -220,39 +236,59 @@
     normal4(philox(c, k0, k1), z);
     return sigma * z[0];
 }
-template <int PP, bool MV>
+template <int PP, bool MV, bool DRAW>
 __global__ __launch_bounds__(256, (MV && PP <= 16) ? 3 : (PP <= 16 ? 2 : 1)) void k_perturb(abc_rng key, const double* __restrict__ theta, size_t K, int P,
                                                  const abc_prior* __restrict__ priors,
                                                  const unsigned long long* __restrict__ parent,
                                                  unsigned long long i0, size_t n,
                                                  const double* __restrict__ L_or_dv , double* __restrict__ out,
-                                                 unsigned long long* __restrict__ giveups) {
+                                                 unsigned long long* __restrict__ giveups, abc_draw_deferred dr,
+                                                 unsigned long long* __restrict__ parent_out) {
     __shared__ double sS[PP];
     __shared__ abc_prior sp[PP];
     __shared__ double sinv[PP];
     if (!MV) for (int p = threadIdx.x; p < PP; p += 256) sS[p] = (p < P) ? sqrt(L_or_dv[p]) : 0.0;
     for (int p = threadIdx.x; p < PP; p += 256) {
         abc_prior q; q.kind = ABC_PRIOR_UNIF_REAL; q.pad_ = 0; q.a = -1e300; q.b = 1e300;
-        sp[p] = (p < P) ? priors[p] : q;
-        sinv[p] = (p < P && priors[p].kind == ABC_PRIOR_GAUSS && fabs(priors[p].b) < 1e10 && fabs(priors[p].b) > 1e-300) ? 1.0 / fabs(priors[p].b) : 0.0;
+        if (p < P) { q.kind = priors[p].kind; q.a = priors[p].a; q.b = priors[p].b; }
+        sp[p] = q;
+        sinv[p] = (p < P && q.kind == ABC_PRIOR_GAUSS && fabs(q.b) < 1e10 && fabs(q.b) > 1e-300) ? 1.0 / fabs(q.b) : 0.0;
     }
     __syncthreads();
     const size_t i = (size_t)blockIdx.x * 256 + threadIdx.x;
+    if (DRAW && i == 0 && dr.verdict_src) publish_verdict(dr.verdict_src, dr.verdict_dev, dr.verdict_pin);
     if (i >= n) return;
     {
     const unsigned long long gi = i0 + i;
-    const double* mrow = theta + (size_t)parent[i] * PP;
+    size_t par = 0, cell = 0;
+    double du = 0.0, dF = 0.0;
+    uint32_t dA = 0u;
+    if constexpr (DRAW && MV) { cell = alias_cell(dr.raw[i], dr.K, &du); dF = dr.F[cell]; dA = dr.A[cell]; }
+    else if constexpr (DRAW) { par = alias_pick(dr.raw[i], dr.F, dr.A, dr.K); parent_out[i] = par; }
+    else par = (size_t)parent[i];
+    const double* mrow = theta + par * PP;
+    double2 m01 = {0.0, 0.0};
+    if constexpr (MV && !DRAW) m01 = *reinterpret_cast<const double2*>(mrow);
     const uint32_t k0 = key.s1 ^ 0x5bd1e995u, k1 = key.s2 ^ (key.s3 * 0x9E3779B1u);
     double x[PP];
     if (MV) {
         for (unsigned attempt = 0; attempt < MVN_MAX_TRIES; attempt++) {
-            mv_noise<PP>(L_or_dv, gi, attempt, k0, k1, x, P);
+            mv_noise<PP>(L_or_dv, gi, attempt, k0, k1, x, P, [&]() {
+                if constexpr (DRAW) {
+                    if (attempt == 0) {
+                        par = alias_choose(du, cell, dF, dA, dr.K);
+                        parent_out[i] = par;
+                        mrow = theta + par * PP;
+                        m01 = *reinterpret_cast<const double2*>(mrow);
+                    }
+                }
+            });
             bool ok = true;
             asm volatile("" ::: "memory");
 #pragma unroll
             for (int a = 0; a < PP; a += 2) {
                 if (PP > 32 && a >= P) continue;
-                const double2 m = *reinterpret_cast<const double2*>(mrow + a);
+                const double2 m = (a == 0) ? m01 : *reinterpret_cast<const double2*>(mrow + a);
                 x[a] = recast_valid(sp[a], sinv[a], x[a] + m.x, ok);
                 x[a + 1] = recast_valid(sp[a + 1], sinv[a + 1], x[a + 1] + m.y, ok);
             }
@@ -560,8 +596,9 @@
 int launch_resample(abc_ctx* ctx, const abc_rng* rng, const double* w, size_t K, uint64_t i0, size_t n,
                     uint64_t* parent, int (*while_host_builds)(void*), void* hook_arg, bool uniform_weights,
                     const uint32_t* raw_ready, bool weights_on_host, const volatile int* abort_flag, bool parents_ready,
-                    int* alias_check_deferred) {
+                    int* alias_check_deferred, abc_draw_deferred* draw_deferred) {
     if (alias_check_deferred) *alias_check_deferred = 0;
+    if (draw_deferred) *draw_deferred = {};
     bool wait_side = raw_ready != nullptr;
     if (n == 0) return ABC_OK;
     if (K == 0 || K > 0xffffffffull) ABC_FAIL(ctx, ABC_ERR_INVALID, "resample: K = %zu", K);
@@ -577,6 +614,7 @@
         else ABC_TRY(taus_stream(ctx, base, n, raw));
         if (while_host_builds) ABC_TRY(while_host_builds(hook_arg));
         if (!(parents_ready && raw_ready)) {
+            if (draw_deferred) { *draw_deferred = {raw, ctx->ualias_F, ctx->ualias_A, K, nullptr, nullptr, nullptr}; return ABC_OK; }
             hipLaunchKernelGGL(k_alias_draw, dim3((unsigned)((n + 255) / 256)), dim3(256), 0, ctx->stream, raw, n, ctx->ualias_F,
                                ctx->ualias_A, K, (unsigned long long*)parent);
             ABC_HIP(ctx, hipGetLastError());
@@ -612,6 +650,11 @@
         }
         ctx->alias_dev_builds++;
         if (while_host_builds) ABC_TRY(while_host_builds(hook_arg));
+        if (draw_deferred && alias_check_deferred) {
+            *draw_deferred = {raw, ctx->alias_F, ctx->alias_A, K, verdict, ctx->alias_fail_dev, fail_pin};
+            *alias_check_deferred = 1;
+            return ABC_OK;
+        }
         {
             StageTimer tm(ctx, ST_RESAMPLE);
             hipLaunchKernelGGL(k_alias_draw, dim3((unsigned)((n + 255) / 256)), dim3(256), 0, ctx->stream, raw, n, ctx->alias_F,
@@ -662,6 +705,7 @@
     }
     StageTimer tm(ctx, ST_RESAMPLE);
     ABC_HIP(ctx, hipMemcpyAsync(ctx->alias_F, hF, K * (sizeof(double) + sizeof(uint32_t)), hipMemcpyHostToDevice, ctx->stream));
+    if (draw_deferred) { *draw_deferred = {raw, ctx->alias_F, ctx->alias_A, K, nullptr, nullptr, nullptr}; return ABC_OK; }
     hipLaunchKernelGGL(k_alias_draw, dim3((unsigned)((n + 255) / 256)), dim3(256), 0, ctx->stream, raw, n, ctx->alias_F,
                        ctx->alias_A, K, (unsigned long long*)parent);
     ABC_HIP(ctx, hipGetLastError());
@@ -728,12 +772,22 @@
 
 int launch_perturb(abc_ctx* ctx, const abc_rng* rng, const double* theta, size_t K, size_t P, const abc_prior* priors,
                    const uint64_t* parent, uint64_t i0, size_t n, int multivariate, const double* L_or_dv, double* out,
-                   uint64_t* seeds, uint64_t seed_stream_offset, const abc_perturb_prep* prep) {
+                   uint64_t* seeds, uint64_t seed_stream_offset, const abc_perturb_prep* prep, const abc_draw_deferred* draw) {
     if (n == 0) return ABC_OK;
     int PP = 2;
     while (PP < (int)P) PP *= 2;
     if (P > 64) PP = (int)((P + 63) / 64 * 64);
     ABC_TRY(abc_giveups_ensure(ctx));
+    bool fused_draw = draw && draw->raw;
+    unsigned long long* parent_out = fused_draw ? (unsigned long long*)const_cast<uint64_t*>(parent) : nullptr;
+    if (fused_draw && (PP > 64 || (PP == 64 && !multivariate))) {
+        StageTimer tr(ctx, ST_RESAMPLE);
+        hipLaunchKernelGGL(k_alias_draw, dim3((unsigned)((n + 255) / 256)), dim3(256), 0, ctx->stream, draw->raw, n, draw->F, draw->A,
+                           draw->K, parent_out, draw->verdict_src, draw->verdict_dev, draw->verdict_pin);
+        ABC_HIP(ctx, hipGetLastError());
+        fused_draw = false;
+    }
+    const abc_draw_deferred dr = fused_draw ? *draw : abc_draw_deferred{};
     StageTimer tm(ctx, ST_PERTURB);
     const unsigned blocks = (unsigned)((n + 255) / 256);
     double* rows = (prep && prep->rows) ? prep->rows : (double*)abc_ws_alloc(ctx, K * (size_t)PP * sizeof(double));
@@ -760,16 +814,14 @@
         if (seeds && !(prep && prep->seeds_done)) ABC_TRY(launch_seeds(ctx, rng, i0, n, seeds, seed_stream_offset, nullptr));
         return ABC_OK;
     }
+#define LAUNCH_PT2(PPV, MVV, DRAWV, LV)                                                                                 \
+    hipLaunchKernelGGL((k_perturb<PPV, MVV, DRAWV>), dim3(blocks), dim3(256), 0, ctx->stream, *rng, theta, K, (int)P,  \
+                       priors, DRAWV ? nullptr : (const unsigned long long*)parent, (unsigned long long)i0, n, LV, out, \
+                       ctx->giveups_dev, dr, parent_out)
 #define LAUNCH_PT(PPV)                                                                                                 \
     do {                                                                                                               \
-        if (multivariate)                                                                                              \
-            hipLaunchKernelGGL((k_perturb<PPV, true>), dim3(blocks), dim3(256), 0, ctx->stream, *rng, theta, K, (int)P, \
-                               priors, (const unsigned long long*)parent, (unsigned long long)i0, n, Lpad, out,       \
-                               ctx->giveups_dev);                                                                     \
-        else                                                                                                           \
-            hipLaunchKernelGGL((k_perturb<PPV, false>), dim3(blocks), dim3(256), 0, ctx->stream, *rng, theta, K, (int)P, \
-                               priors, (const unsigned long long*)parent, (unsigned long long)i0, n, L_or_dv, out,    \
-                               ctx->giveups_dev);                                                                     \
+        if (multivariate) { if (fused_draw) LAUNCH_PT2(PPV, true, true, Lpad); else LAUNCH_PT2(PPV, true, false, Lpad); } \
+        else { if (fused_draw) LAUNCH_PT2(PPV, false, true, L_or_dv); else LAUNCH_PT2(PPV, false, false, L_or_dv); }   \
     } while (0)
     switch (PP) {
         case 2: LAUNCH_PT(2); break;
@@ -789,6 +841,7 @@
             break;
     }
 #undef LAUNCH_PT
+#undef LAUNCH_PT2
     ABC_HIP(ctx, hipGetLastError());
     if (seeds && !(prep && prep->seeds_done)) ABC_TRY(launch_seeds(ctx, rng, i0, n, seeds, seed_stream_offset, nullptr));
     return ABC_OK;
diff --git a/abcsmc_amd/csrc/sharded.hip b/abcsmc_amd/csrc/sharded.hip
--- a/abcsmc_amd/csrc/sharded.hip
+++ b/abcsmc_amd/csrc/sharded.hip
@@ -701,14 +701,15 @@
         if (moments_on_side) ABC_HIP(ctx, hipStreamWaitEvent(ctx->stream, ctx->ev_moments, 0));
         abc_prep_arg pa = {ctx, rng, theta, theta_stats, K, P, Nn, cfg->next0, cfg->Nnext_total, io->seeds, &prep, moments_on_side ? nullptr : L,
                            spd_dev, dv, false, nullptr, nullptr, nullptr};
+        abc_draw_deferred draw = {};
         {
             const int rc = launch_resample(ctx, rng, io->w, K, cfg->next0, Nn, parent, abc_prep_hook, &pa, uniform_w, raw_early, w_on_host,
-                                           (ds_fail_dev && !uniform_w) ? pfail_early : nullptr, false, &alias_deferred);
+                                           (ds_fail_dev && !uniform_w) ? pfail_early : nullptr, false, &alias_deferred, &draw);
             if (rc == ABC_INTERNAL_RETRY) return repeat_with_radix();
             ABC_TRY(rc);
         }
         ABC_TRY(launch_perturb(ctx, rng, theta, K, P, io->priors, parent, cfg->next0, Nn, cfg->multivariate,
-                               cfg->multivariate ? L : dv, io->next, io->seeds, cfg->Nnext_total, &prep));
+                               cfg->multivariate ? L : dv, io->next, io->seeds, cfg->Nnext_total, &prep, &draw));
         parent_used = parent; L_used = L; prep_used = prep;
     } else if (cfg->multivariate && io->L) {
         have_spd = true;
```
